# ska-telescope/ska-sdp-screen-fitting

Measured on AMD Instinct MI355X. Metric: screen-slots/sec (ant×time×freq) + FITS-cube wall-clock, KL 256² screen, higher is better.
Workload: dtype f64

## Files before the change

### include/screenfit.h

```cpp
#ifndef SCREENFIT_H
#define SCREENFIT_H

#include <stddef.h>
#include <stdint.h>

#ifdef __cplusplus
extern "C" {
#endif

#define SF_OK 0
#define SF_EINVAL (-22)
#define SF_ENOMEM (-12)
#define SF_EIO (-5)
#define SF_ENODEV (-19)

#define SF_MAX_DIR 60
#define SF_MAX_FIT_DIR 128
#define SF_MAX_EVAL_DIR 128

#define SF_SCREEN_PHASE 0
#define SF_SCREEN_TEC 1
#define SF_SCREEN_AMPLITUDE 2

#define SF_EVAL_NAN_SCRUB 1u
#define SF_EVAL_FAST_SINCOS (1u << 8)
#define SF_EVAL_NT_STORES (1u << 9)
#define SF_EVAL_BIG_ENDIAN (1u << 10)

typedef struct sf_ctx sf_ctx;

typedef struct sf_fit_params {
  int screen_type;
  int niter;
  double nsigma;
  int adjust_order;
  int ref_ant;
  int ant_offset;
  const double* ref_phase;
} sf_fit_params;

const char* sf_version(void);
const char* sf_last_error(void);
int sf_create(int device, sf_ctx** out);
int sf_destroy(sf_ctx* ctx);
int sf_set_stream(sf_ctx* ctx, void* hip_stream);
int sf_synchronize(sf_ctx* ctx);
int sf_stream_create(sf_ctx* ctx, const int* reserve_cus, int n_reserve,
                     void** hip_stream);
int sf_stream_destroy(sf_ctx* ctx, void* hip_stream);
int sf_device_cus(sf_ctx* ctx, int* n_cu);
#define SF_OPT_FIT_GENERAL 1
#define SF_OPT_EVAL_KERNEL 2
#define SF_OPT_EVAL_MAX_BLOCKS 3
#define SF_OPT_FIT_PACK 4
#define SF_OPT_EVAL_KS_PAD 5
#define SF_OPT_EVAL_SLEEP 6
#define SF_OPT_EVAL_XCD_MAP 7
#define SF_OPT_EVAL_GROUPS 8
#define SF_OPT_EVAL_BANDS 9
#define SF_OPT_FIT_LEAN 10
#define SF_OPT_TESS_SLOTS 11
#define SF_OPT_TESS_WAVES 12
#define SF_OPT_TESS_TILE 13
#define SF_OPT_TESS_BOX 14
#define SF_OPT_EVAL_INT 15
#define SF_OPT_EVAL_WG_WAVES 16
#define SF_OPT_FIT_EIG_WAVES 17
#define SF_OPT_FIT_SUBSET_DELETION 18
#define SF_OPT_FIT_WIDE_CACHE 19
#define SF_OPT_FIT_WIDE_POOL_MB 20
#define SF_OPT_FIT_WIDE_POOL_MAX 21
#define SF_OPT_FIT_LANE 22
#define SF_EVAL_KERNEL_AUTO 0
#define SF_EVAL_KERNEL_TILE 1
#define SF_EVAL_KERNEL_LDS4 2
#define SF_EVAL_KERNEL_LDS8 3
#define SF_EVAL_KERNEL_LDS16 4
#define SF_EVAL_KERNEL_LDS8H 5
#define SF_EVAL_KERNEL_LDS16H 6
#define SF_EVAL_KERNEL_TILE3 7
#define SF_EVAL_KERNEL_SHB 8
#define SF_EVAL_KERNEL_WIDE 9
int sf_get_eval_kernel(sf_ctx* ctx, int gain, unsigned flags, int* kernel);
#define SF_EVAL_CONTRACTION_F64 0
#define SF_EVAL_CONTRACTION_I8_DIGITS 1
int sf_get_eval_contraction(sf_ctx* ctx, int gain, unsigned flags, int* contraction);
int sf_set_option(sf_ctx* ctx, int option, int value);
int sf_alloc(sf_ctx* ctx, size_t bytes, void** dev_ptr);
int sf_free(sf_ctx* ctx, void* dev_ptr);
int sf_copy_h2d(sf_ctx* ctx, void* dst_dev, const void* src_host, size_t bytes);
int sf_copy_d2h(sf_ctx* ctx, void* dst_host, const void* src_dev, size_t bytes);

int sf_set_basis(sf_ctx* ctx, const double* pp_host, int D, double r0,
                 double beta);
int sf_set_basis_wide(sf_ctx* ctx, const double* pp_host, int D, double r0,
                      double beta);
int sf_get_basis(sf_ctx* ctx, double* c_host, double* pinv_c_host,
                 double* u_host, double* eig_host);

int sf_set_piercepoints(sf_ctx* ctx, const double* pp_host, int D, double r0,
                        double beta);

int sf_kl_fit(sf_ctx* ctx, const double* phase, const float* weight, int T,
              int F, int A, const int* station_order_host,
              const sf_fit_params* params, double* coef, double* resid,
              float* w_out, int32_t* order_out);

int sf_get_fit_stats(sf_ctx* ctx, int* n_masks, int* n_general);

int sf_get_fit_lane_stats(sf_ctx* ctx, int64_t* n_lane, int64_t* n_deferred);

int sf_get_fit_pool(sf_ctx* ctx, uint64_t* masks_host, double* entries_host,
                    int max_masks, int* n_masks);
int sf_get_fit_pool_wide(sf_ctx* ctx, uint64_t* masks_host, double* entries_host,
                         int max_masks, int* n_masks);

int sf_set_grid(sf_ctx* ctx, const double* x_host, int nx,
                const double* y_host, int ny);

int sf_kl_eval(sf_ctx* ctx, const double* coef, int64_t S, float* out,
               int64_t ring_slots, unsigned flags);

int sf_kl_eval_gain(sf_ctx* ctx, const double* coef_phase,
                    const double* coef_xx, const double* coef_yy, int64_t S,
                    float* out, int64_t ring_slots, unsigned flags);
int sf_kl_eval_sums(sf_ctx* ctx, const double* coef_phase,
                    const double* coef_xx, const double* coef_yy, int64_t S,
                    float* out, int64_t ring, unsigned flags,
                    uint32_t* slot_sums);

int sf_kl_eval_values(sf_ctx* ctx, const double* coef, int64_t S, float* out,
                      int64_t ring_slots, unsigned flags);

int sf_kl_eval_pol(sf_ctx* ctx, const double* phase_xx, const double* phase_yy,
                   const double* amp_xx, const double* amp_yy, int64_t S,
                   float* out, int64_t ring_slots, unsigned flags);

#define SF_MAX_TEC_FREQ 4096
int sf_set_tec_freqs(sf_ctx* ctx, const double* rad_per_tecu_host,
                     const int* tec_index_host, int F, int F_tec);
int sf_kl_eval_tec(sf_ctx* ctx, const double* tec_coef, const double* phase_coef,
                   int64_t T, int A, float* out, unsigned flags);

#define SF_MAX_POINTS 4096
int sf_set_points(sf_ctx* ctx, const double* xy_host, int P);
int sf_kl_eval_points(sf_ctx* ctx, const double* coef_phase, const double* coef_xx,
                      const double* coef_yy, int64_t S, float* planes, unsigned flags);
int sf_kl_eval_point_values(sf_ctx* ctx, const double* coef, int64_t S, double* values);

int sf_tess_fill(sf_ctx* ctx, const int32_t* labels, int nx, int ny,
                 const double* phase, const double* amp_xx,
                 const double* amp_yy, int D, int64_t S, float* out,
                 int64_t ring_slots, double smooth_pix, unsigned flags);
int sf_tess_fill_pol(sf_ctx* ctx, const int32_t* labels, int nx, int ny,
                     const double* phase, const double* phase_yy,
                     const double* amp_xx, const double* amp_yy, int D, int64_t S,
                     float* out, int64_t ring_slots, double smooth_pix,
                     unsigned flags);

int sf_smooth(sf_ctx* ctx, float* cube, int nx, int ny, int64_t n_img,
              double smooth_pix, unsigned flags);

#ifdef __cplusplus
}
#endif
#endif
```

### ska-sdp-screen-fitting_amd/csrc/capi.hip

```cpp
#include <hip/hip_runtime.h>

#include <algorithm>
#include <cmath>
#include <cstring>
#include <string>
#include <vector>

#include "sf_internal.h"

namespace sf {
static thread_local std::string g_last_error;
void set_error(const std::string& msg) { g_last_error = msg; }
}

using sf::set_error;

namespace {

int check_device(int device) {
  int n = 0;
  hipError_t e = hipGetDeviceCount(&n);
  if (e != hipSuccess || n == 0) {
    set_error("no HIP device available");
    return SF_ENODEV;
  }
  if (device < 0 || device >= n) {
    set_error("device index out of range");
    return SF_EINVAL;
  }
  hipDeviceProp_t prop;
  SF_HIP(hipGetDeviceProperties(&prop, device));
  if (std::strncmp(prop.gcnArchName, "gfx950", 6) != 0) {
    set_error(std::string("libscreenfit is built for gfx950, found ") +
              prop.gcnArchName);
    return SF_ENODEV;
  }
  return SF_OK;
}

template <typename T>
int rebind(sf::DevBuf<T>& b, size_t count) {
  b.reset();
  return b.reserve(count, "hipMalloc failed");
}

void drop_wide(sf_ctx* ctx) {
  ctx->wide = 0;
  ctx->d_wide_ws.reset();
  ctx->d_wkeys.reset();
  ctx->d_wslot.reset();
  ctx->d_wtab.reset();
  ctx->d_wtab_id.reset();
  ctx->d_wpool_mask.reset();
  ctx->d_wpool.reset();
  ctx->wide_pool_n = 0;
}

void drop_geometry(sf_ctx* ctx) {
  ctx->D = 0;
  ctx->has_basis = 0;
  drop_wide(ctx);
  ctx->nx = ctx->ny = 0;
  ctx->n_pix = 0;
  ctx->n_points = 0;
}

}

extern "C" {

const char* sf_version(void) { return "screenfit 0.1.0 (gfx950)"; }

const char* sf_last_error(void) { return sf::g_last_error.c_str(); }

int sf_create(int device, sf_ctx** out) {
  SF_REQUIRE(out != nullptr, SF_EINVAL, "sf_create: out is NULL");
  SF_TRY(check_device(device));
  SF_HIP(hipSetDevice(device));
  sf_ctx* ctx = new sf_ctx();
  ctx->device = device;
  if (ctx->d_trash.reserve(256, "sf_create: hipMalloc failed") != SF_OK) {
    delete ctx;
    return SF_ENOMEM;
  }
  *out = ctx;
  return SF_OK;
}

int sf_destroy(sf_ctx* ctx) {
  if (!ctx) return SF_OK;
  hipSetDevice(ctx->device);
  if (ctx->kdig_read) (void)hipEventDestroy(ctx->kdig_read);
  delete ctx;
  return SF_OK;
}

int sf_set_stream(sf_ctx* ctx, void* stream) {
  SF_REQUIRE(ctx, SF_EINVAL, "sf_set_stream: NULL context");
  ctx->stream = reinterpret_cast<hipStream_t>(stream);
  return SF_OK;
}

int sf_device_cus(sf_ctx* ctx, int* n_cu) {
  SF_REQUIRE(ctx && n_cu, SF_EINVAL, "sf_device_cus: NULL argument");
  SF_HIP(hipDeviceGetAttribute(n_cu, hipDeviceAttributeMultiprocessorCount,
                               ctx->device));
  return SF_OK;
}

int sf_stream_create(sf_ctx* ctx, const int* reserve_cus, int n_reserve,
                     void** stream) {
  SF_REQUIRE(ctx && stream && n_reserve >= 0 && (n_reserve == 0 || reserve_cus),
             SF_EINVAL, "sf_stream_create: bad argument");
  SF_HIP(hipSetDevice(ctx->device));
  int n_cu = 0;
  SF_TRY(sf_device_cus(ctx, &n_cu));
  hipStream_t s = nullptr;
  if (n_reserve == 0) {
    SF_HIP(hipStreamCreateWithFlags(&s, hipStreamNonBlocking));
  } else {
    std::vector<uint32_t> mask((n_cu + 31) / 32, 0u);
    for (int c = 0; c < n_cu; ++c) mask[c >> 5] |= 1u << (c & 31);
    for (int k = 0; k < n_reserve; ++k) {
      const int c = reserve_cus[k];
      SF_REQUIRE(c >= 0 && c < n_cu, SF_EINVAL, "sf_stream_create: CU index out of range");
      mask[c >> 5] &= ~(1u << (c & 31));
    }
    SF_REQUIRE(n_reserve < n_cu, SF_EINVAL, "sf_stream_create: no CU left");
    SF_HIP(hipExtStreamCreateWithCUMask(&s, (uint32_t)mask.size(), mask.data()));
  }
  *stream = s;
  return SF_OK;
}

int sf_stream_destroy(sf_ctx* ctx, void* stream) {
  SF_REQUIRE(ctx && stream, SF_EINVAL, "sf_stream_destroy: bad argument");
  SF_HIP(hipSetDevice(ctx->device));
  SF_HIP(hipStreamDestroy(reinterpret_cast<hipStream_t>(stream)));
  return SF_OK;
}

int sf_set_option(sf_ctx* ctx, int option, int value) {
  SF_REQUIRE(ctx, SF_EINVAL, "sf_set_option: NULL context");
  switch (option) {
    case SF_OPT_FIT_GENERAL:
      ctx->force_general = value != 0;
      return SF_OK;
    case SF_OPT_EVAL_KERNEL:
      SF_REQUIRE(value >= SF_EVAL_KERNEL_AUTO && value <= SF_EVAL_KERNEL_WIDE,
                 SF_EINVAL, "sf_set_option: unknown evaluation kernel");
      ctx->eval_kernel = value;
      return SF_OK;
    case SF_OPT_FIT_PACK:
      ctx->fit_pack = value != 0;
      return SF_OK;
    case SF_OPT_FIT_LEAN:
      ctx->fit_lean = value != 0;
      return SF_OK;
    case SF_OPT_FIT_LANE:
      ctx->fit_lane = value != 0;
      return SF_OK;
    case SF_OPT_EVAL_KS_PAD:
      SF_REQUIRE(value >= 0 && value <= 3, SF_EINVAL,
                 "sf_set_option: k-step padding must be 0..3");
      ctx->eval_ks_pad = value;
      return SF_OK;
    case SF_OPT_EVAL_SLEEP:
      SF_REQUIRE(value >= 0 && value <= 1000, SF_EINVAL,
                 "sf_set_option: eval sleep must be 0..1000");
      ctx->eval_sleep = value;
      return SF_OK;
    case SF_OPT_EVAL_XCD_MAP:
      SF_REQUIRE(value >= -1 && value <= 1, SF_EINVAL,
                 "sf_set_option: XCD map must be -1, 0 or 1");
      ctx->eval_xcd_map = value;
      return SF_OK;
    case SF_OPT_EVAL_GROUPS:
      SF_REQUIRE(value >= 0 && value <= 256 && (value & (value - 1)) == 0,
                 SF_EINVAL, "sf_set_option: groups must be 0 or a power of two <= 256");
      ctx->eval_groups = value;
      return SF_OK;
    case SF_OPT_EVAL_BANDS:
      SF_REQUIRE(value >= 0 && value <= 128 && (value & (value - 1)) == 0,
                 SF_EINVAL, "sf_set_option: bands must be 0 or a power of two <= 128");
      ctx->eval_bands = value;
      return SF_OK;
    case SF_OPT_TESS_SLOTS:
      SF_REQUIRE(value >= 0 && value <= 256, SF_EINVAL,
                 "sf_set_option: tess slots must be 0..256");
      ctx->tess_slots = value;
      return SF_OK;
    case SF_OPT_TESS_TILE:
      SF_REQUIRE(value == 0 || value == 1, SF_EINVAL, "sf_set_option: tess tile must be 0 or 1");
      ctx->tess_tile = value;
      return SF_OK;
    case SF_OPT_TESS_BOX:
      SF_REQUIRE(value >= -1 && value <= 1, SF_EINVAL,
                 "sf_set_option: tess box must be -1, 0 or 1");
      ctx->tess_box = value;
      return SF_OK;
    case SF_OPT_TESS_WAVES:
      SF_REQUIRE(value == 0 || value == 4 || value == 8 || value == 16, SF_EINVAL,
                 "sf_set_option: tess waves must be 0, 4, 8 or 16");
      ctx->tess_waves = value;
      return SF_OK;
    case SF_OPT_EVAL_MAX_BLOCKS:
      SF_REQUIRE(value >= 0, SF_EINVAL, "sf_set_option: negative block cap");
      ctx->eval_max_blocks = value;
      return SF_OK;
    case SF_OPT_EVAL_INT:
      SF_REQUIRE(value == -1 || value == 0, SF_EINVAL,
                 "sf_set_option: eval int must be -1 or 0");
      ctx->eval_int = value;
      return SF_OK;
    case SF_OPT_EVAL_WG_WAVES:
      SF_REQUIRE(value == 0 || value == 4 || value == 8, SF_EINVAL,
                 "sf_set_option: eval workgroup waves must be 0, 4 or 8");
      ctx->eval_wg_waves = value;
      return SF_OK;
    case SF_OPT_FIT_SUBSET_DELETION:
      SF_REQUIRE(value >= 0 && value <= 3, SF_EINVAL,
                 "SF_OPT_FIT_SUBSET_DELETION must be 0, 1, 2 or 3");
      ctx->fit_subset_deletion = (int)value;
      return SF_OK;
    case SF_OPT_FIT_EIG_WAVES:
      SF_REQUIRE(value >= 0 && value <= 4, SF_EINVAL,
                 "sf_set_option: fit eig waves must be 0..4");
      ctx->fit_eig_waves = value;
      return SF_OK;
    case SF_OPT_FIT_WIDE_CACHE:
      SF_REQUIRE(value == 0 || value == 1, SF_EINVAL,
                 "sf_set_option: fit wide cache must be 0 or 1");
      ctx->wide_cache = value;
      return SF_OK;
    case SF_OPT_FIT_WIDE_POOL_MB:
      SF_REQUIRE(value >= 0 && value <= 65536, SF_EINVAL,
                 "sf_set_option: fit wide pool MiB must be 0..65536");
      ctx->wide_pool_mb = value;
      return SF_OK;
    case SF_OPT_FIT_WIDE_POOL_MAX:
      SF_REQUIRE(value >= 0, SF_EINVAL,
                 "sf_set_option: negative fit wide pool entry cap");
      ctx->wide_pool_max = value;
      return SF_OK;
    default:
      set_error("sf_set_option: unknown option");
      return SF_EINVAL;
  }
}

int sf_get_eval_kernel(sf_ctx* ctx, int gain, unsigned flags, int* kernel) {
  SF_REQUIRE(ctx && kernel, SF_EINVAL, "sf_get_eval_kernel: bad argument");
  SF_REQUIRE(ctx->ksteps > 0, SF_EINVAL,
             "sf_get_eval_kernel: call sf_set_grid first");
  *kernel = sf::pick_eval_kernel(ctx, gain != 0, flags, true);
  return SF_OK;
}

int sf_get_eval_contraction(sf_ctx* ctx, int gain, unsigned flags, int* contraction) {
  SF_REQUIRE(ctx && contraction, SF_EINVAL, "sf_get_eval_contraction: bad argument");
  SF_REQUIRE(ctx->ksteps > 0, SF_EINVAL,
             "sf_get_eval_contraction: call sf_set_grid first");
  *contraction = sf::eval_int_applies(ctx, gain != 0, flags, true)
                     ? SF_EVAL_CONTRACTION_I8_DIGITS
                     : SF_EVAL_CONTRACTION_F64;
  return SF_OK;
}

int sf_synchronize(sf_ctx* ctx) {
  SF_REQUIRE(ctx, SF_EINVAL, "sf_synchronize: NULL context");
  SF_HIP(hipSetDevice(ctx->device));
  SF_HIP(hipStreamSynchronize(ctx->stream));
  return SF_OK;
}

int sf_alloc(sf_ctx* ctx, size_t bytes, void** p) {
  SF_REQUIRE(ctx && p, SF_EINVAL, "sf_alloc: bad argument");
  SF_HIP(hipSetDevice(ctx->device));
  if (hipMalloc(p, bytes) != hipSuccess) {
    set_error("sf_alloc: hipMalloc failed");
    return SF_ENOMEM;
  }
  return SF_OK;
}

int sf_free(sf_ctx* ctx, void* p) {
  SF_REQUIRE(ctx, SF_EINVAL, "sf_free: NULL context");
  SF_HIP(hipSetDevice(ctx->device));
  SF_HIP(hipFree(p));
  return SF_OK;
}

int sf_copy_h2d(sf_ctx* ctx, void* dst, const void* src, size_t bytes) {
  SF_REQUIRE(ctx && (bytes == 0 || (dst && src)), SF_EINVAL,
             "sf_copy_h2d: bad argument");
  SF_HIP(hipSetDevice(ctx->device));
  SF_HIP(hipMemcpyAsync(dst, src, bytes, hipMemcpyHostToDevice, ctx->stream));
  SF_HIP(hipStreamSynchronize(ctx->stream));
  return SF_OK;
}

int sf_copy_d2h(sf_ctx* ctx, void* dst, const void* src, size_t bytes) {
  SF_REQUIRE(ctx && (bytes == 0 || (dst && src)), SF_EINVAL,
             "sf_copy_d2h: bad argument");
  SF_HIP(hipSetDevice(ctx->device));
  SF_HIP(hipMemcpyAsync(dst, src, bytes, hipMemcpyDeviceToHost, ctx->stream));
  SF_HIP(hipStreamSynchronize(ctx->stream));
  return SF_OK;
}

int sf_set_basis(sf_ctx* ctx, const double* pp, int D, double r0,
                 double beta) {
  SF_REQUIRE(ctx && pp, SF_EINVAL, "sf_set_basis: bad argument");
  SF_REQUIRE(D >= 1 && D <= SF_MAX_DIR, SF_EINVAL,
             "sf_set_basis: D out of range [1, SF_MAX_DIR]");
  SF_REQUIRE(r0 > 0.0, SF_EINVAL, "sf_set_basis: r0 must be > 0");
  SF_HIP(hipSetDevice(ctx->device));
  SF_HIP(hipStreamSynchronize(ctx->stream));
  drop_geometry(ctx);
  SF_TRY(rebind(ctx->d_pp, (size_t)3 * D));
  SF_TRY(rebind(ctx->d_c, (size_t)D * D));
  SF_TRY(rebind(ctx->d_pinv, (size_t)D * D));
  SF_TRY(rebind(ctx->d_u, (size_t)D * D));
  SF_TRY(rebind(ctx->d_eig, (size_t)64));
  SF_HIP(hipMemcpy(ctx->d_pp, pp, sizeof(double) * 3 * D,
                   hipMemcpyHostToDevice));
  for (int i = 0; i < 3 * D; ++i) ctx->h_pp[i] = pp[i];
  SF_HIP(hipMemset(ctx->d_eig, 0, 64 * sizeof(double)));
  ctx->D = D;
  ctx->r0 = r0;
  ctx->beta = beta;
  int rc = sf::launch_basis(ctx);
  if (rc == SF_OK && hipStreamSynchronize(ctx->stream) != hipSuccess) {
    set_error("sf_set_basis: basis kernel failed");
    rc = SF_EIO;
  }
  if (rc != SF_OK) ctx->D = 0;
  ctx->has_basis = rc == SF_OK;
  return rc;
}

int sf_set_piercepoints(sf_ctx* ctx, const double* pp, int D, double r0,
                        double beta) {
  SF_REQUIRE(ctx && pp, SF_EINVAL, "sf_set_piercepoints: bad argument");
  SF_REQUIRE(D >= 1 && D <= SF_MAX_EVAL_DIR, SF_EINVAL,
             "sf_set_piercepoints: D out of range [1, SF_MAX_EVAL_DIR]");
  SF_REQUIRE(r0 > 0.0, SF_EINVAL, "sf_set_piercepoints: r0 must be > 0");
  SF_HIP(hipSetDevice(ctx->device));
  SF_HIP(hipStreamSynchronize(ctx->stream));
  drop_geometry(ctx);
  SF_TRY(rebind(ctx->d_pp, (size_t)3 * D));
  SF_HIP(hipMemcpy(ctx->d_pp, pp, sizeof(double) * 3 * D,
                   hipMemcpyHostToDevice));
  for (int i = 0; i < 3 * D; ++i) ctx->h_pp[i] = pp[i];
  ctx->D = D;
  ctx->r0 = r0;
  ctx->beta = beta;
  return SF_OK;
}

int sf_set_basis_wide(sf_ctx* ctx, const double* pp, int D, double r0,
                      double beta) {
  SF_REQUIRE(ctx && pp, SF_EINVAL, "sf_set_basis_wide: bad argument");
  SF_REQUIRE(D >= 1 && D <= SF_MAX_FIT_DIR, SF_EINVAL,
             "sf_set_basis_wide: D out of range [1, SF_MAX_FIT_DIR]");
  if (D <= SF_MAX_DIR) return sf_set_basis(ctx, pp, D, r0, beta);
  SF_TRY(sf_set_piercepoints(ctx, pp, D, r0, beta));
  drop_geometry(ctx);
  SF_TRY(rebind(ctx->d_c, (size_t)D * D));
  SF_TRY(rebind(ctx->d_pinv, (size_t)D * D));
  SF_TRY(rebind(ctx->d_u, (size_t)D * D));
  SF_TRY(rebind(ctx->d_eig, (size_t)SF_MAX_FIT_DIR));
  SF_HIP(hipMemset(ctx->d_eig, 0, SF_MAX_FIT_DIR * sizeof(double)));
  ctx->D = D;
  int rc = sf::launch_basis_wide(ctx);
  if (rc == SF_OK && hipStreamSynchronize(ctx->stream) != hipSuccess) {
    set_error("sf_set_basis_wide: basis kernel failed");
    rc = SF_EIO;
  }
  if (rc != SF_OK) ctx->D = 0;
  ctx->has_basis = rc == SF_OK;
  ctx->wide = rc == SF_OK;
  return rc;
}

int sf_get_basis(sf_ctx* ctx, double* c, double* pinv, double* u,
                 double* eig) {
  SF_REQUIRE(ctx && ctx->D > 0, SF_EINVAL, "sf_get_basis: no basis set");
  SF_REQUIRE(ctx->has_basis, SF_EINVAL,
             "sf_get_basis: the context holds piercepoints only "
             "(sf_set_piercepoints); call sf_set_basis");
  SF_HIP(hipSetDevice(ctx->device));
  SF_HIP(hipStreamSynchronize(ctx->stream));
  const size_t n = (size_t)ctx->D * ctx->D * sizeof(double);
  if (c) SF_HIP(hipMemcpy(c, ctx->d_c, n, hipMemcpyDeviceToHost));
  if (pinv) SF_HIP(hipMemcpy(pinv, ctx->d_pinv, n, hipMemcpyDeviceToHost));
  if (u) SF_HIP(hipMemcpy(u, ctx->d_u, n, hipMemcpyDeviceToHost));
  if (eig)
    SF_HIP(hipMemcpy(eig, ctx->d_eig, ctx->D * sizeof(double),
                     hipMemcpyDeviceToHost));
  return SF_OK;
}

int sf_kl_fit(sf_ctx* ctx, const double* phase, const float* weight, int T,
              int F, int A, const int* st_order, const sf_fit_params* p,
              double* coef, double* resid, float* w_out, int32_t* order_out) {
  SF_REQUIRE(ctx && ctx->D > 0, SF_EINVAL, "sf_kl_fit: call sf_set_basis first");
  SF_REQUIRE(ctx->has_basis, SF_EINVAL,
             "sf_kl_fit: the context holds piercepoints only "
             "(sf_set_piercepoints); the fit needs sf_set_basis");
  SF_REQUIRE(phase && weight && st_order && p && coef, SF_EINVAL,
             "sf_kl_fit: NULL argument");
  SF_REQUIRE(T >= 1 && F >= 1 && A >= 1, SF_EINVAL,
             "sf_kl_fit: T, F, A must be >= 1");
  SF_REQUIRE((int64_t)F * A <= INT32_MAX / 2, SF_EINVAL,
             "sf_kl_fit: F * A too large");
  SF_REQUIRE(p->screen_type == SF_SCREEN_PHASE || p->screen_type == SF_SCREEN_TEC ||
                 p->screen_type == SF_SCREEN_AMPLITUDE,
             SF_EINVAL, "sf_kl_fit: unsupported screen type");
  SF_REQUIRE(p->niter >= 1 && p->niter <= 64, SF_EINVAL,
             "sf_kl_fit: niter must be in [1, 64]");
  SF_REQUIRE((int64_t)T * F * A * (2 * p->niter + 2) < ((int64_t)1 << 30),
             SF_EINVAL,
             "sf_kl_fit: too many slots for one call (split the time axis)");
  SF_REQUIRE(p->ref_ant >= -1 && p->ant_offset >= 0, SF_EINVAL,
             "sf_kl_fit: bad ref_ant / ant_offset");
  {
    const int rl = p->ref_ant - p->ant_offset;
    SF_REQUIRE(p->ref_ant == -1 || p->ref_phase || (rl >= 0 && rl < A),
               SF_EINVAL,
               "sf_kl_fit: reference station not in this shard and no "
               "ref_phase given");
  }
  for (int a = 0; a < A; ++a)
    SF_REQUIRE(st_order[a] >= 0, SF_EINVAL, "sf_kl_fit: negative order");
  SF_HIP(hipSetDevice(ctx->device));
  SF_TRY(ctx->d_skip.reserve((size_t)F * A, "hipMalloc failed"));
  SF_TRY(ctx->d_st_order.reserve((size_t)A, "hipMalloc failed"));
  SF_HIP(hipMemcpyAsync(ctx->d_st_order, st_order, sizeof(int) * A,
                        hipMemcpyHostToDevice, ctx->stream));
  return sf::launch_fit(ctx, phase, weight, T, F, A, p, coef, resid, w_out,
                        order_out);
}

int sf_get_fit_stats(sf_ctx* ctx, int* n_masks, int* n_general) {
  SF_REQUIRE(ctx, SF_EINVAL, "sf_get_fit_stats: NULL context");
  int c[sf::kFitCounters] = {};
  SF_HIP(hipSetDevice(ctx->device));
  SF_HIP(hipStreamSynchronize(ctx->stream));
  if (ctx->d_counters)
    SF_HIP(hipMemcpy(c, ctx->d_counters, sizeof(c), hipMemcpyDeviceToHost));
  static_assert(sf::kCntIds == sf::kCntWideDecomp, "n_masks reads one slot");
  if (n_masks) *n_masks = c[sf::kCntIds];
  if (n_general) *n_general = c[sf::kCntSlow];
  return SF_OK;
}

int sf_get_fit_lane_stats(sf_ctx* ctx, int64_t* n_lane, int64_t* n_deferred) {
  SF_REQUIRE(ctx, SF_EINVAL, "sf_get_fit_lane_stats: NULL context");
  int c[sf::kFitCounters] = {};
  SF_HIP(hipSetDevice(ctx->device));
  SF_HIP(hipStreamSynchronize(ctx->stream));
  if (ctx->d_counters)
    SF_HIP(hipMemcpy(c, ctx->d_counters, sizeof(c), hipMemcpyDeviceToHost));
  if (n_lane) *n_lane = c[sf::kCntLane];
  if (n_deferred) *n_deferred = c[sf::kCntLaneDeferred];
  return SF_OK;
}

int sf_get_fit_pool(sf_ctx* ctx, uint64_t* masks_host, double* entries_host,
                    int max_masks, int* n_masks) {
  SF_REQUIRE(ctx && n_masks && max_masks >= 0, SF_EINVAL, "sf_get_fit_pool: bad argument");
  SF_REQUIRE(max_masks == 0 || (masks_host && entries_host), SF_EINVAL,
             "sf_get_fit_pool: NULL output");
  SF_REQUIRE(!ctx->wide, SF_EINVAL,
             "sf_get_fit_pool: 64-bit mask keys; above SF_MAX_DIR directions "
             "(sf_set_basis_wide) call sf_get_fit_pool_wide");
  SF_HIP(hipSetDevice(ctx->device));
  SF_HIP(hipStreamSynchronize(ctx->stream));
  int c0 = 0;
  if (ctx->d_counters)
    SF_HIP(hipMemcpy(&c0, ctx->d_counters + sf::kCntIds, sizeof(int),
                     hipMemcpyDeviceToHost));
  const int n = ctx->pool_D == ctx->D && (size_t)c0 <= ctx->d_pool_mask.size() ? c0 : 0;
  *n_masks = n;
  const int k = n < max_masks ? n : max_masks;
  if (k > 0) {
    const size_t entry = (size_t)ctx->D * ctx->D + ctx->D;
    SF_HIP(hipMemcpy(masks_host, ctx->d_pool_mask, k * sizeof(uint64_t),
                     hipMemcpyDeviceToHost));
    SF_HIP(hipMemcpy(entries_host, ctx->d_pool, k * entry * sizeof(double),
                     hipMemcpyDeviceToHost));
  }
  return SF_OK;
}

int sf_get_fit_pool_wide(sf_ctx* ctx, uint64_t* masks_host, double* entries_host,
                         int max_masks, int* n_masks) {
  SF_REQUIRE(ctx && n_masks && max_masks >= 0, SF_EINVAL,
             "sf_get_fit_pool_wide: bad argument");
  SF_REQUIRE(max_masks == 0 || (masks_host && entries_host), SF_EINVAL,
             "sf_get_fit_pool_wide: NULL output");
  SF_REQUIRE(ctx->wide && ctx->has_basis, SF_EINVAL,
             "sf_get_fit_pool_wide: the context holds no wide basis "
             "(sf_set_basis_wide with more than SF_MAX_DIR directions)");
  SF_HIP(hipSetDevice(ctx->device));
  SF_HIP(hipStreamSynchronize(ctx->stream));
  const int n = ctx->wide_pool_n;
  *n_masks = n;
  const int k = n < max_masks ? n : max_masks;
  if (k > 0) return sf::read_fit_pool_wide(ctx, masks_host, entries_host, k);
  return SF_OK;
}

int sf_set_grid(sf_ctx* ctx, const double* x, int nx, const double* y,
                int ny) {
  SF_REQUIRE(ctx && ctx->D > 0, SF_EINVAL,
             "sf_set_grid: call sf_set_basis or sf_set_piercepoints first");
  SF_REQUIRE(x && y && nx >= 1 && ny >= 1, SF_EINVAL, "sf_set_grid: bad grid");
  for (int i = 0; i < nx; ++i)
    SF_REQUIRE(std::isfinite(x[i]), SF_EINVAL, "sf_set_grid: non-finite x coordinate");
  for (int j = 0; j < ny; ++j)
    SF_REQUIRE(std::isfinite(y[j]), SF_EINVAL, "sf_set_grid: non-finite y coordinate");
  SF_REQUIRE((int64_t)nx * ny <= ((int64_t)1 << 31), SF_EINVAL,
             "sf_set_grid: grid too large");
  SF_HIP(hipSetDevice(ctx->device));
  ctx->n_pix = 0;
  ctx->nx = nx;
  ctx->ny = ny;
  const int64_t n_pix = (int64_t)nx * ny;
  ctx->n_pix_blocks = (n_pix + sf::kBlockPix - 1) / sf::kBlockPix;
  ctx->ksteps = (ctx->D + 3) / 4;
  const size_t n = (size_t)ctx->n_pix_blocks * sf::kEvalWaves * ctx->ksteps *
                   sf::kTiles * 64;
  SF_TRY(rebind(ctx->d_cfrag, n));
  sf::DevBuf<double> dx, dy;
  sf::DevBuf<int> dbad;
  SF_TRY(dx.reserve((size_t)nx, "hipMalloc failed"));
  SF_TRY(dy.reserve((size_t)ny, "hipMalloc failed"));
  int rc = SF_OK;
  if (hipMemcpyAsync(dx, x, sizeof(double) * nx, hipMemcpyHostToDevice,
                     ctx->stream) != hipSuccess ||
      hipMemcpyAsync(dy, y, sizeof(double) * ny, hipMemcpyHostToDevice,
                     ctx->stream) != hipSuccess) {
    set_error("sf_set_grid: copy of the grid coordinates failed");
    rc = SF_EIO;
  } else {
    rc = sf::launch_cpix(ctx, dx, dy);
  }
  double cmax = 0.0;
  for (int d = 0; d < ctx->D; ++d) {
    const double px = ctx->h_pp[3 * d], py = ctx->h_pp[3 * d + 1];
    double mx = 0.0, my = 0.0, nxd = HUGE_VAL, nyd = HUGE_VAL;
    for (int i = 0; i < nx; ++i) {
      mx = std::fmax(mx, std::fabs(px - x[i]));
      nxd = std::fmin(nxd, std::fabs(px - x[i]));
    }
    for (int j = 0; j < ny; ++j) {
      my = std::fmax(my, std::fabs(py - y[j]));
      nyd = std::fmin(nyd, std::fabs(py - y[j]));
    }
    const double z = ctx->h_pp[3 * d + 2];
    for (const double d2 : {mx * mx + my * my + z * z, nxd * nxd + nyd * nyd + z * z}) {
      const double c = 1.01 * 0.5 * std::pow(d2 / (ctx->r0 * ctx->r0), ctx->beta / 2.0);
      cmax = std::isfinite(c) ? std::fmax(cmax, c) : HUGE_VAL;
    }
  }
  ctx->dig_ok = 0;
  if (rc == SF_OK && ctx->ksteps >= 12 && ctx->ksteps <= sf::kEvalMaxKS &&
      std::isfinite(cmax) &&
      cmax * 68719476736.0 < std::ldexp(1.0, 46) * 1.86) {
    if (rebind(ctx->d_cdig, (size_t)ctx->n_pix_blocks * sf::kEvalWaves * sf::kDigits *
                                sf::kTiles * 64 * 16) == SF_OK &&
        dbad.reserve(1, "hipMalloc failed") == SF_OK &&
        hipMemsetAsync(dbad, 0, sizeof(int), ctx->stream) == hipSuccess) {
      rc = sf::launch_cdig(ctx, dx, dy, dbad);
      if (rc == SF_OK) ctx->dig_ok = 1;
    }
  }
  if (hipStreamSynchronize(ctx->stream) != hipSuccess && rc == SF_OK) {
    set_error("sf_set_grid: pixel basis kernel failed");
    rc = SF_EIO;
  }
  if (ctx->dig_ok) {
    int bad = 1;
    if (hipMemcpy(&bad, dbad, sizeof(int), hipMemcpyDeviceToHost) != hipSuccess || bad)
      ctx->dig_ok = 0;
  }
  if (rc == SF_OK) {
    ctx->rev_thr = cmax > 0.0 && std::isfinite(cmax) ? 32768.0 / cmax : 0.0;
    ctx->n_pix = n_pix;
  } else {
    ctx->dig_ok = 0;
  }
  return rc;
}

int sf_kl_eval(sf_ctx* ctx, const double* coef, int64_t S, float* out,
               int64_t ring, unsigned flags) {
  SF_REQUIRE(ctx && ctx->n_pix > 0 && ctx->d_cfrag, SF_EINVAL,
             "sf_kl_eval: call sf_set_grid first");
  SF_REQUIRE(coef && out && S >= 0 && ring >= 1, SF_EINVAL,
             "sf_kl_eval: bad argument");
  if (S == 0) return SF_OK;
  SF_HIP(hipSetDevice(ctx->device));
  return sf::launch_eval(ctx, coef, nullptr, nullptr, S, out, ring, flags,
                         nullptr);
}

int sf_kl_eval_gain(sf_ctx* ctx, const double* coef_phase,
                    const double* coef_xx, const double* coef_yy, int64_t S,
                    float* out, int64_t ring, unsigned flags) {
  SF_REQUIRE(ctx && ctx->n_pix > 0 && ctx->d_cfrag, SF_EINVAL,
             "sf_kl_eval_gain: call sf_set_grid first");
  SF_REQUIRE(coef_phase && coef_xx && coef_yy && out && S >= 0 && ring >= 1,
             SF_EINVAL, "sf_kl_eval_gain: bad argument");
  if (S == 0) return SF_OK;
  SF_HIP(hipSetDevice(ctx->device));
  return sf::launch_eval(ctx, coef_phase, coef_xx, coef_yy, S, out, ring, flags,
                         nullptr);
}

int sf_kl_eval_sums(sf_ctx* ctx, const double* coef_phase,
                    const double* coef_xx, const double* coef_yy, int64_t S,
                    float* out, int64_t ring, unsigned flags,
                    uint32_t* slot_sums) {
  SF_REQUIRE(ctx && ctx->n_pix > 0 && ctx->d_cfrag, SF_EINVAL,
             "sf_kl_eval_sums: call sf_set_grid first");
  SF_REQUIRE(coef_phase && out && slot_sums && S >= 0 && ring >= 1,
             SF_EINVAL, "sf_kl_eval_sums: bad argument");
  SF_REQUIRE((coef_xx == nullptr) == (coef_yy == nullptr), SF_EINVAL,
             "sf_kl_eval_sums: give both amplitude coefficient sets or neither");
  if (S == 0) return SF_OK;
  SF_HIP(hipSetDevice(ctx->device));
  return sf::launch_eval(ctx, coef_phase, coef_xx, coef_yy, S, out, ring, flags,
                         reinterpret_cast<unsigned*>(slot_sums));
}

int sf_set_points(sf_ctx* ctx, const double* xy, int P) {
  SF_REQUIRE(ctx, SF_EINVAL, "sf_set_points: NULL context");
  SF_REQUIRE(ctx->D > 0, SF_EINVAL,
             "sf_set_points: call sf_set_basis, sf_set_basis_wide or "
             "sf_set_piercepoints first");
  SF_REQUIRE(xy, SF_EINVAL, "sf_set_points: NULL positions");
  SF_REQUIRE(P >= 1 && P <= SF_MAX_POINTS, SF_EINVAL,
             "sf_set_points: P out of range [1, SF_MAX_POINTS]");
  for (int i = 0; i < 2 * P; ++i)
    SF_REQUIRE(std::isfinite(xy[i]), SF_EINVAL, "sf_set_points: non-finite coordinate");
  SF_HIP(hipSetDevice(ctx->device));
  SF_HIP(hipStreamSynchronize(ctx->stream));
  ctx->n_points = 0;
  if (ctx->pt_cus == 0) SF_TRY(sf_device_cus(ctx, &ctx->pt_cus));
  const int tiles = sf::points_tiles(P), ks_pad = sf::points_ks_pad(ctx->D);
  SF_TRY(rebind(ctx->d_pxy, (size_t)2 * P));
  SF_TRY(rebind(ctx->d_pfrag, (size_t)tiles * ks_pad * 64));
  SF_HIP(hipMemcpy(ctx->d_pxy, xy, sizeof(double) * 2 * P, hipMemcpyHostToDevice));
  ctx->pt_tiles = tiles;
  ctx->pt_ks_pad = ks_pad;
  ctx->n_points = P;
  int rc = sf::launch_points_cpix(ctx);
  if (rc == SF_OK && hipStreamSynchronize(ctx->stream) != hipSuccess) {
    set_error("sf_set_points: point basis kernel failed");
    rc = SF_EIO;
  }
  if (rc != SF_OK) ctx->n_points = 0;
  return rc;
}

int sf_kl_eval_points(sf_ctx* ctx, const double* coef_phase, const double* coef_xx,
                      const double* coef_yy, int64_t S, float* planes,
                      unsigned flags) {
  SF_REQUIRE(ctx, SF_EINVAL, "sf_kl_eval_points: NULL context");
  SF_REQUIRE(ctx->D > 0 && ctx->n_points > 0 && ctx->d_pfrag, SF_EINVAL,
             "sf_kl_eval_points: call sf_set_points first");
  SF_REQUIRE(coef_phase && planes, SF_EINVAL, "sf_kl_eval_points: NULL argument");
  SF_REQUIRE((coef_xx == nullptr) == (coef_yy == nullptr), SF_EINVAL,
             "sf_kl_eval_points: give both amplitude coefficient sets or neither");
  SF_REQUIRE(S >= 1, SF_EINVAL, "sf_kl_eval_points: S must be >= 1");
  SF_REQUIRE((flags & ~(SF_EVAL_NAN_SCRUB | SF_EVAL_FAST_SINCOS)) == 0, SF_EINVAL,
             "sf_kl_eval_points: flags other than SF_EVAL_NAN_SCRUB and "
             "SF_EVAL_FAST_SINCOS");
  SF_HIP(hipSetDevice(ctx->device));
  return sf::launch_eval_points(ctx, coef_phase, coef_xx, coef_yy, S, planes, flags);
}

int sf_kl_eval_point_values(sf_ctx* ctx, const double* coef, int64_t S,
                            double* values) {
  SF_REQUIRE(ctx, SF_EINVAL, "sf_kl_eval_point_values: NULL context");
  SF_REQUIRE(ctx->D > 0 && ctx->n_points > 0 && ctx->d_pfrag, SF_EINVAL,
             "sf_kl_eval_point_values: call sf_set_points first");
  SF_REQUIRE(coef && values, SF_EINVAL, "sf_kl_eval_point_values: NULL argument");
  SF_REQUIRE(S >= 1, SF_EINVAL, "sf_kl_eval_point_values: S must be >= 1");
  SF_HIP(hipSetDevice(ctx->device));
  return sf::launch_eval_point_values(ctx, coef, S, values);
}

int sf_kl_eval_values(sf_ctx* ctx, const double* coef, int64_t S, float* out,
                      int64_t ring, unsigned flags) {
  SF_REQUIRE(ctx, SF_EINVAL, "sf_kl_eval_values: NULL context");
  SF_REQUIRE(ctx->D > 0 && ctx->n_pix > 0 && ctx->d_cfrag, SF_EINVAL,
             "sf_kl_eval_values: call sf_set_grid first");
  SF_REQUIRE(coef && out && S >= 0 && ring >= 1, SF_EINVAL,
             "sf_kl_eval_values: bad argument");
  SF_REQUIRE((reinterpret_cast<uintptr_t>(out) & 3) == 0, SF_EINVAL,
             "sf_kl_eval_values: output not 4-byte aligned");
  SF_REQUIRE((flags & ~(SF_EVAL_NAN_SCRUB | SF_EVAL_NT_STORES | SF_EVAL_BIG_ENDIAN)) == 0,
             SF_EINVAL,
             "sf_kl_eval_values: flags other than SF_EVAL_NAN_SCRUB, "
             "SF_EVAL_NT_STORES and SF_EVAL_BIG_ENDIAN");
  if (S == 0) return SF_OK;
  SF_HIP(hipSetDevice(ctx->device));
  return sf::launch_eval_values(ctx, coef, S, out, ring, flags);
}

int sf_kl_eval_pol(sf_ctx* ctx, const double* phase_xx, const double* phase_yy,
                   const double* amp_xx, const double* amp_yy, int64_t S, float* out,
                   int64_t ring, unsigned flags) {
  SF_REQUIRE(ctx, SF_EINVAL, "sf_kl_eval_pol: NULL context");
  SF_REQUIRE(ctx->D > 0 && ctx->n_pix > 0 && ctx->d_cfrag, SF_EINVAL,
             "sf_kl_eval_pol: call sf_set_grid first");
  SF_REQUIRE(phase_xx && phase_yy, SF_EINVAL,
             "sf_kl_eval_pol: both phase coefficient sets are required");
  SF_REQUIRE((amp_xx == nullptr) == (amp_yy == nullptr), SF_EINVAL,
             "sf_kl_eval_pol: give both amplitude coefficient sets or neither");
  SF_REQUIRE(out && S >= 0 && ring >= 1, SF_EINVAL, "sf_kl_eval_pol: bad argument");
  SF_REQUIRE((reinterpret_cast<uintptr_t>(out) & 3) == 0, SF_EINVAL,
             "sf_kl_eval_pol: output not 4-byte aligned");
  SF_REQUIRE((flags & ~(SF_EVAL_NAN_SCRUB | SF_EVAL_FAST_SINCOS | SF_EVAL_NT_STORES |
                        SF_EVAL_BIG_ENDIAN)) == 0,
             SF_EINVAL,
             "sf_kl_eval_pol: flags other than SF_EVAL_NAN_SCRUB, SF_EVAL_FAST_SINCOS, "
             "SF_EVAL_NT_STORES and SF_EVAL_BIG_ENDIAN");
  if (S == 0) return SF_OK;
  SF_HIP(hipSetDevice(ctx->device));
  return sf::launch_eval_pol(ctx, phase_xx, phase_yy, amp_xx, amp_yy, S, out, ring, flags);
}

int sf_set_tec_freqs(sf_ctx* ctx, const double* rad_per_tecu, const int* tec_index,
                     int F, int F_tec) {
  SF_REQUIRE(ctx, SF_EINVAL, "sf_set_tec_freqs: NULL context");
  SF_REQUIRE(rad_per_tecu, SF_EINVAL, "sf_set_tec_freqs: NULL scales");
  SF_REQUIRE(F >= 1 && F <= SF_MAX_TEC_FREQ, SF_EINVAL,
             "sf_set_tec_freqs: F out of range [1, SF_MAX_TEC_FREQ]");
  SF_REQUIRE(F_tec >= 1, SF_EINVAL, "sf_set_tec_freqs: F_tec must be >= 1");
  for (int f = 0; f < F; ++f) {
    SF_REQUIRE(std::isfinite(rad_per_tecu[f]), SF_EINVAL,
               "sf_set_tec_freqs: non-finite scale");
    SF_REQUIRE(!tec_index || (tec_index[f] >= 0 && tec_index[f] < F_tec), SF_EINVAL,
               "sf_set_tec_freqs: TEC frequency index out of range [0, F_tec)");
  }
  std::vector<double> k(F);
  std::vector<int> ch(F), order(F);
  for (int f = 0; f < F; ++f) order[f] = f;
  std::stable_sort(order.begin(), order.end(), [&](int a, int b) {
    return (tec_index ? tec_index[a] : 0) < (tec_index ? tec_index[b] : 0);
  });
  std::vector<int> used, off(1, 0);
  for (int c = 0; c < F; ++c) {
    const int f = order[c], i = tec_index ? tec_index[f] : 0;
    if (used.empty() || used.back() != i) {
      if (!used.empty()) off.push_back(c);
      used.push_back(i);
    }
    k[c] = rad_per_tecu[f] / 6.283185307179586;
    ch[c] = f;
  }
  off.push_back(F);
  SF_HIP(hipSetDevice(ctx->device));
  SF_HIP(hipStreamSynchronize(ctx->stream));
  sf::DevBuf<double> d;
  SF_TRY(d.reserve((size_t)F + (F + 1) / 2, "sf_set_tec_freqs: hipMalloc failed"));
  if (hipMemcpy(d, k.data(), F * sizeof(double), hipMemcpyHostToDevice) != hipSuccess ||
      hipMemcpy(d + F, ch.data(), F * sizeof(int), hipMemcpyHostToDevice) != hipSuccess) {
    set_error("sf_set_tec_freqs: copy of the channel lists failed");
    return SF_EIO;
  }
  ctx->d_tec_ch.swap(d);
  ctx->tec_F = F;
  ctx->tec_F_tec = F_tec;
  ctx->tec_used.swap(used);
  ctx->tec_off.swap(off);
  return SF_OK;
}

int sf_kl_eval_tec(sf_ctx* ctx, const double* tec_coef, const double* phase_coef,
                   int64_t T, int A, float* out, unsigned flags) {
  SF_REQUIRE(ctx, SF_EINVAL, "sf_kl_eval_tec: NULL context");
  SF_REQUIRE(ctx->D > 0 && ctx->n_pix > 0 && ctx->d_cfrag, SF_EINVAL,
             "sf_kl_eval_tec: call sf_set_grid first");
  SF_REQUIRE(ctx->tec_F > 0 && ctx->d_tec_ch, SF_EINVAL,
             "sf_kl_eval_tec: call sf_set_tec_freqs first");
  SF_REQUIRE(tec_coef && out && T >= 0 && A >= 1, SF_EINVAL,
             "sf_kl_eval_tec: bad argument");
  SF_REQUIRE(T * A <= INT32_MAX, SF_EINVAL,
             "sf_kl_eval_tec: T * A too large for one call (split the time axis)");
  SF_REQUIRE((reinterpret_cast<uintptr_t>(out) & 3) == 0, SF_EINVAL,
             "sf_kl_eval_tec: output not 4-byte aligned");
  SF_REQUIRE((flags & ~(SF_EVAL_NAN_SCRUB | SF_EVAL_FAST_SINCOS | SF_EVAL_NT_STORES |
                        SF_EVAL_BIG_ENDIAN)) == 0,
             SF_EINVAL,
             "sf_kl_eval_tec: flags other than SF_EVAL_NAN_SCRUB, SF_EVAL_FAST_SINCOS, "
             "SF_EVAL_NT_STORES and SF_EVAL_BIG_ENDIAN");
  if (T == 0) return SF_OK;
  SF_HIP(hipSetDevice(ctx->device));
  return sf::launch_eval_tec(ctx, tec_coef, phase_coef, T, A, out, flags);
}

static int upload_gaussian(sf_ctx* ctx, double sigma, int* R_out) {
  if (sigma <= 1e-15) sigma = 0.0;
  const int R = sigma > 0.0 ? (int)(4.0 * sigma + 0.5) : 0;
  *R_out = R;
  if (ctx->d_gw && sigma == ctx->gw_sigma) return SF_OK;
  std::vector<double> w(1, 1.0);
  if (sigma > 0.0) {
    w.assign(2 * R + 1, 0.0);
    double sum = 0.0;
    for (int i = -R; i <= R; ++i)
      w[i + R] = std::exp(-0.5 / (sigma * sigma) * (double)(i * i));
    for (int i = 0; i < 2 * R + 1; ++i) sum += w[i];
    for (int i = 0; i < 2 * R + 1; ++i) w[i] /= sum;
  }
  SF_HIP(hipDeviceSynchronize());
  ctx->gw_sigma = -1.0;
  SF_TRY(ctx->d_gw.reserve(w.size() < 64 ? 64 : w.size(), "hipMalloc failed"));
  SF_HIP(hipMemcpyAsync(ctx->d_gw, w.data(), w.size() * sizeof(double),
                        hipMemcpyHostToDevice, ctx->stream));
  SF_HIP(hipStreamSynchronize(ctx->stream));
  ctx->gw_sigma = sigma;
  return SF_OK;
}

int sf_tess_fill(sf_ctx* ctx, const int32_t* labels, int nx, int ny,
                 const double* phase, const double* amp_xx,
                 const double* amp_yy, int D, int64_t S, float* out,
                 int64_t ring, double smooth_pix, unsigned flags) {
  return sf_tess_fill_pol(ctx, labels, nx, ny, phase, nullptr, amp_xx, amp_yy, D, S, out, ring,
                          smooth_pix, flags);
}

int sf_tess_fill_pol(sf_ctx* ctx, const int32_t* labels, int nx, int ny,
                     const double* phase, const double* phase_yy, const double* amp_xx,
                     const double* amp_yy, int D, int64_t S, float* out,
                     int64_t ring, double smooth_pix, unsigned flags) {
  SF_REQUIRE(ctx && labels && phase && out, SF_EINVAL, "sf_tess_fill: NULL argument");
  SF_REQUIRE(nx >= 1 && ny >= 1 && D >= 1 && D <= SF_MAX_EVAL_DIR && S >= 0 && ring >= 1 &&
                 ring <= INT32_MAX,
             SF_EINVAL, "sf_tess_fill: bad shape");
  SF_REQUIRE(smooth_pix >= 0.0 && smooth_pix <= 1e4, SF_EINVAL,
             "sf_tess_fill: smooth_pix must be in [0, 1e4]");
  if (S == 0) return SF_OK;
  SF_HIP(hipSetDevice(ctx->device));
  int R = 0;
  int rc = upload_gaussian(ctx, smooth_pix, &R);
  if (rc != SF_OK) return rc;
  if (R <= sf::kTessMaxR)
    return (ctx->tess_tile ? sf::launch_tess_tile : sf::launch_tess)(
        ctx, labels, nx, ny, phase, phase_yy, amp_xx, amp_yy, D, S, out, ring, ctx->d_gw, R,
        flags);
  SF_REQUIRE(ring >= S, SF_EINVAL,
             "sf_tess_fill: smooth_pix > 6 needs ring_slots >= S");
  rc = sf::launch_tess(ctx, labels, nx, ny, phase, phase_yy, amp_xx, amp_yy, D, S, out,
                       ring, ctx->d_gw, 0, 0u);
  if (rc != SF_OK) return rc;
  return sf::launch_smooth(ctx, out, nx, ny, S * 4, ctx->d_gw, R, flags);
}

int sf_smooth(sf_ctx* ctx, float* cube, int nx, int ny, int64_t n_img,
              double smooth_pix, unsigned flags) {
  SF_REQUIRE(ctx && cube && nx >= 1 && ny >= 1 && n_img >= 0, SF_EINVAL,
             "sf_smooth: bad argument");
  SF_REQUIRE(n_img % 4 == 0, SF_EINVAL,
             "sf_smooth: n_img must count whole [4][ny][nx] slot cubes");
  SF_REQUIRE(smooth_pix >= 0.0 && smooth_pix <= 1e4, SF_EINVAL,
             "sf_smooth: smooth_pix must be in [0, 1e4]");
  if (n_img == 0) return SF_OK;
  SF_HIP(hipSetDevice(ctx->device));
  int R = 0;
  const int rc = upload_gaussian(ctx, smooth_pix, &R);
  if (rc != SF_OK) return rc;
  return sf::launch_smooth(ctx, cube, nx, ny, n_img, ctx->d_gw, R, flags);
}

}
```

### ska-sdp-screen-fitting_amd/csrc/kl_fit_fast.hip

```cpp
#include <hip/hip_runtime.h>

#include <cmath>
#include <cstdlib>

#include "kl_fit_lane.h"
#include "kl_fit_pool.h"
#include "kl_fit_steps.h"
#include "sf_internal.h"

namespace sf {

constexpr size_t kLdsBytes = 160 * 1024;
constexpr double kTinyW = kPinvAtol * 1.001;

template <int GW>
__global__ __launch_bounds__(256) void kl_classify_kernel(
    const float* __restrict__ weight, int64_t S, int F, int A, int D,
    const int* __restrict__ st_order, const uint8_t* __restrict__ skip,
    int ref_skip, unsigned long long* __restrict__ keys, int cap,
    int* __restrict__ pos, uint8_t* __restrict__ cls,
    int* __restrict__ counters,
    double* __restrict__ coef, double* __restrict__ resid,
    float* __restrict__ w_out, int32_t* __restrict__ order_out, int lane_fit) {
  constexpr int kPerWave = 64 / GW;
  const int l = lane();
  const int g = l / GW;
  const int d = l % GW;
  const int64_t s = ((int64_t)blockIdx.x * (blockDim.x / 64) + threadIdx.x / 64) *
                        kPerWave + g;
  const bool live = s < S && d < D;
  float x = 0.0f;
  if (live) {
    x = weight[s * D + d];
    w_out[s * D + d] = x;
  }
  const unsigned long long bm = __ballot(live && x > 0.0f);
  const unsigned long long bt = __ballot(live && x > 0.0f && (double)x <= kTinyW);
  const unsigned long long gmask = (GW == 64) ? ~0ull : ((1ull << GW) - 1ull);
  const unsigned long long mask = (bm >> (g * GW)) & gmask;
  const bool tiny = ((bt >> (g * GW)) & gmask) != 0ull;
  const float w_first = __shfl(x, g * GW + (mask ? __builtin_ctzll(mask) : 0));
  const unsigned long long bn = __ballot(live && x > 0.0f && x != w_first);
  const bool nonuniform = ((bn >> (g * GW)) & gmask) != 0ull;
  if (s >= S) return;
  const SlotGeom sg(s, F, A);
  const bool skipped = sg.skipped(skip, ref_skip);
  if (live && skipped) {
    coef[s * D + d] = 0.0;
    resid[s * D + d] = 0.0;
  }
  if (d != 0) return;
  if (skipped) {
    cls[s] = kClassSkipped;
    order_out[s] = 0;
    pos[s] = -2;
    return;
  }
  order_out[s] = st_order[sg.a];
  if (tiny) atomicAdd(counters + kCntSlow, 1);
  else if (nonuniform) atomicAdd(counters + kCntNonUniform, 1);
  const bool to_lane = lane_fit && !tiny && !nonuniform && mask == full_mask(D);
  cls[s] = tiny ? kClassSlow : to_lane ? kClassLane : kClassFast;
  if (mask == full_mask(D)) pos[s] = -1;
  else if (mask == 0ull) pos[s] = -2;
  else pos[s] = table_insert(keys, cap, mask);
}

struct FastLds {
  const double* U;
  const double* C;
  int cld;
  const double* lam;
  double* Vs;
  double* lams;
  double* G;
  double* M;
  double* vec;
  double2* cs;
  int2* pr;
  __device__ void jacobi(double* a, double* v, int n, int ld) const {
    wave_jacobi(a, v, cs, pr, n, ld, kJacobiMaxSweeps);
  }
};

__host__ __device__ inline size_t fast_shared_bytes(int D, bool c_global) {
  return (size_t)((c_global ? 1 : 2) * D * odd_ld(D) + 64) * sizeof(double);
}
__host__ __device__ inline size_t fast_wave_bytes(int D, bool slow, bool lean = false) {
  if (lean) return (size_t)6 * 64 * sizeof(double);
  return (size_t)((slow ? 3 : 2) * D * odd_ld(D) + 64 + 6 * 64) * sizeof(double) +
         (slow ? 64 * sizeof(double2) + 96 * sizeof(int2) : 0);
}

struct Basis {
  int n;
  bool full;
  int ld;
  const double* U;
  const double* lam;
};

template <bool SLOW, int SPW, bool LEAN>
__device__ void fit_once(const FastLds& L, const Basis& B, int D, int ld,
                         int K, int screen_type, bool uniform, double wu,
                         double phi_p, double w_p, double phi_d, double w_d,
                         double& white_d, double& resid_d) {
#pragma clang fp contract(off)
  using G = Group<SPW>;
  using M = FitMath<!SLOW>;
  constexpr int kMatVecUnroll = LEAN ? 4 : 1;
  const int l = G::lane();
  const int n = B.n;
  double* v0 = L.vec;
  double* v1 = L.vec + 64;
  double* v2 = L.vec + 128;
  double* v3 = L.vec + 192;
  double rc = 0.0, rs = 0.0;
  if (l < n) {
    if (screen_type == SF_SCREEN_PHASE) {
      double sn, cn;
      M::sin_cos(phi_p, &sn, &cn);
      rc = w_p * cn;
      rs = w_p * sn;
    } else if (screen_type == SF_SCREEN_AMPLITUDE) {
      rc = w_p * M::lg10(phi_p);
    } else {
      rc = w_p * phi_p;
    }
    v0[l] = rc;
    v1[l] = rs;
    v2[l] = w_p;
  }
  lds_sync();
  const Tie2 tie(n, K, v0, v1, v2, B.lam);
  double a1 = 0.0, a2 = 0.0;
  if (l < K) {
#pragma unroll kMatVecUnroll
    for (int p = 0; p < n; ++p) {
      const double u = B.U[p * B.ld + l];
      a1 += u * v0[p];
      a2 += u * v1[p];
    }
  }
  if (K > 0) {
    if (!SLOW && (LEAN || uniform)) {
      a1 /= wu;
      a2 /= wu;
    } else {
      if (l < K) {
        for (int j = 0; j < K; ++j) {
          double s = 0.0;
          for (int p = 0; p < n; ++p)
            s += B.U[p * B.ld + l] * (v2[p] * B.U[p * B.ld + j]);
          L.G[l * ld + j] = s;
        }
      }
      lds_sync();
      if (!SLOW) {
        wave_cholesky_solve2<SPW>(L.G, K, ld, a1, a2);
      } else {
        truncated_eig_solve(G{}, L, L.G, L.M, K, ld, v0, v1, v2, v3, a1, a2);
      }
    }
  }
  lds_sync();
  if (l < K) {
    const bool keep = fabs(B.lam[l]) > kPinvAtol;
    v0[l] = keep ? a1 : 0.0;
    v1[l] = keep ? a2 : 0.0;
  }
  lds_sync();
  double screen = 0.0;
  if (l < n) {
    double cre = 0.0, cim = 0.0;
#pragma unroll kMatVecUnroll
    for (int k = 0; k < K; ++k) {
      const double u = B.U[l * B.ld + k];
      cre += u * v0[k];
      cim += u * v1[k];
    }
    screen = (screen_type == SF_SCREEN_PHASE) ? M::arctan2(cim, cre) : cre;
    if (tie.on) screen = tie.template screen<M>(screen_type, l);
  }
  lds_sync();
  if (l < n) v2[l] = screen;
  lds_sync();
  if (l < n) {
    double sh = 0.0;
#pragma unroll kMatVecUnroll
    for (int p = 0; p < n; ++p) sh += B.U[p * B.ld + l] * v2[p];
    const double lm = B.lam[l];
    const bool keep = fabs(lm) > kPinvAtol;
    v0[l] = keep ? sh / lm : 0.0;
    v1[l] = keep ? sh : 0.0;
  }
  lds_sync();
  double white = 0.0, cw = 0.0;
  if (l < n) {
#pragma unroll kMatVecUnroll
    for (int r = 0; r < n; ++r) {
      const double u = B.U[l * B.ld + r];
      white += u * v0[r];
      cw += u * v1[r];
    }
  }
  lds_sync();
  if (B.full) {
    white_d = white;
    resid_d = phi_d - model_value<M>(screen_type, cw);
    return;
  }
  if (l < n) {
    v0[l] = screen;
    v1[l] = white;
  }
  lds_sync();
  const bool unfl = (l < D) && (w_d > 0.0);
  const unsigned long long m = G::ballot(unfl);
  double sall = 0.0;
  if (l < D) {
    if (unfl) {
      const int p = G::rank(m);
      sall = v0[p];
    } else {
      unsigned long long mm = m;
      int p = 0;
      while (mm) {
        const int q = __builtin_ctzll(mm);
        sall += L.C[l * L.cld + q] * v1[p];
        mm &= mm - 1;
        ++p;
      }
    }
  }
  lds_sync();
  if (l < D) v2[l] = sall;
  lds_sync();
  if (l < D) {
    double sh = 0.0;
#pragma unroll kMatVecUnroll
    for (int p = 0; p < D; ++p) sh += L.U[p * ld + l] * v2[p];
    const double lm = L.lam[l];
    v0[l] = fabs(lm) > kPinvAtol ? sh / lm : 0.0;
  }
  lds_sync();
  double wa = 0.0;
  if (l < D)
#pragma unroll kMatVecUnroll
    for (int r = 0; r < D; ++r) wa += L.U[l * ld + r] * v0[r];
  lds_sync();
  white_d = wa;
  resid_d = phi_d - model_value<M>(screen_type, sall);
}

#ifndef SF_FIT_MINW
#define SF_FIT_MINW 4
#endif
template <bool SLOW, int SPW, bool LEAN>
__global__ __launch_bounds__(256, SLOW ? 1 : SF_FIT_MINW) void kl_fit_pass_kernel(
    int it, int niter, int64_t S, int F, int A, int D,
    const double* __restrict__ phase, const double* __restrict__ refph,
    int ref_sub, const double* __restrict__ g_u, const double* __restrict__ g_c,
    const double* __restrict__ g_eig, const int* __restrict__ st_order,
    const uint8_t* __restrict__ cls, int* __restrict__ pos,
    const int* __restrict__ ids, unsigned long long* __restrict__ keys, int cap,
    const double* __restrict__ pool, int pool_cap, int* __restrict__ counters,
    int screen_type, double nsigma, int adjust_order, double* __restrict__ coef,
    double* __restrict__ resid, float* __restrict__ w_out,
    int32_t* __restrict__ order_out, const long long* __restrict__ list) {
#pragma clang fp contract(off)
  extern __shared__ double smem[];
  const int ld = odd_ld(D);
  using G = Group<SPW>;
  using M = FitMath<!SLOW>;
  const G tm;
  constexpr bool CG = SPW == 1;
  const int nwaves = blockDim.x / 64;
  const int nslots = nwaves * SPW;
  const int wv = (threadIdx.x / 64) * SPW + G::index();
  const int d = G::lane();
  double* sU = smem;
  double* sC = CG ? nullptr : sU + D * ld;
  double* sl = sU + (CG ? 1 : 2) * D * ld;
  for (int e = threadIdx.x; e < D * D; e += blockDim.x) {
    const int r = e / D, c = e % D;
    sU[r * ld + c] = g_u[e];
    if (!CG) sC[r * ld + c] = g_c[e];
  }
  for (int e = threadIdx.x; e < 64; e += blockDim.x) sl[e] = e < D ? g_eig[e] : 0.0;
  __syncthreads();
  FastLds L;
  L.U = sU;
  L.C = CG ? g_c : sC;
  L.cld = CG ? D : ld;
  L.lam = sl;
  double* wb = sl + 64 + (size_t)wv * (fast_wave_bytes(D, SLOW, LEAN) / sizeof(double));
  if (LEAN) {
    L.Vs = L.G = L.M = L.lams = nullptr;
    L.vec = wb;
    L.cs = nullptr;
    L.pr = nullptr;
  } else {
    L.Vs = wb;
    L.G = wb + D * ld;
    L.M = L.G + D * ld;
    L.lams = (SLOW ? L.M + D * ld : L.G + D * ld);
    L.vec = L.lams + 64;
    L.cs = reinterpret_cast<double2*>(L.vec + 6 * 64);
    L.pr = reinterpret_cast<int2*>(L.cs + 64);
  }
  const uint8_t want = SLOW ? 2 : 0;

  const int64_t n_work = list ? (int64_t)counters[kCntList] : S;
  for (int64_t i = (int64_t)blockIdx.x * nslots + wv; i < n_work;
       i += (int64_t)gridDim.x * nslots) {
    int64_t s = i;
    if (list) {
      const long long e = list[i];
      if (list_first(e) > it) continue;
      s = list_slot(e);
    }
    if (SLOW && cls[s] != want) continue;
    const uint8_t cl = SLOW ? want : cls[s];
    const int a = (int)(s % A);
    const int p0 = pos[s];
    const int64_t base = s * D;
    double phi_d = 0.0, w_d = 0.0, white_d = 0.0, resid_d = 0.0;
    if (d < D) {
      phi_d = phase_ref(phase, refph, ref_sub, s, a, A, D, d);
      w_d = (double)w_out[base + d];
      white_d = it == 0 ? 0.0 : coef[base + d];
      resid_d = it == 0 ? 0.0 : resid[base + d];
    }
    double order = (double)order_out[s];
    const double station_order = (double)st_order[a];
    if (cl != want) continue;
    int id = -1;
    if (p0 >= 0) {
      id = ids[p0];
      if (id < 0 || id >= pool_cap) {
        if (d == 0) atomicOr(counters + kCntError, kErrLookupMiss);
        continue;
      }
    } else if (p0 == -3) {
      if (d == 0) atomicOr(counters + kCntError, kErrTableFull);
      continue;
    }
    const bool unfl = (d < D) && (w_d > 0.0);
    const unsigned long long um = G::ballot(unfl);
    const int n_unfl = __popcll(um);

    Basis B;
    B.n = n_unfl;
    B.full = (n_unfl == D);
    B.ld = ld;
    if (B.full) {
      B.U = L.U;
      B.lam = L.lam;
    } else if (n_unfl > 0) {
      const double* e = pool + (size_t)id * (D * D + D);
      if (LEAN) {
        B.U = e;
        B.ld = D;
        B.lam = e + D * D;
      } else {
        for (int r = 0; r < n_unfl; ++r)
          if (d < n_unfl) L.Vs[r * ld + d] = e[r * D + d];
        if (d < n_unfl) L.lams[d] = e[D * D + d];
        lds_sync();
        B.U = L.Vs;
        B.lam = L.lams;
      }
    }
    double phi_p = 0.0, w_p = 0.0;
    {
      double* v4 = L.vec + 256;
      double* v5 = L.vec + 320;
      if (unfl) {
        const int p = G::rank(um);
        v4[p] = phi_d;
        v5[p] = w_d;
      }
      lds_sync();
      if (d < n_unfl) {
        phi_p = v4[d];
        w_p = v5[d];
      }
      lds_sync();
    }
    const double wmax = G::max(unfl ? w_d : -INFINITY);
    const double wmin = -G::max(unfl ? -w_d : -INFINITY);
    const bool uniform = (wmax == wmin);
    if (LEAN && n_unfl > 0 && !uniform) {
      if (d == 0) atomicOr(counters + kCntError, kErrLeanNonUniform);
      continue;
    }

    if (n_unfl > 0) {
      if (order > n_unfl - 1) order = n_unfl - 1;
      if (it == 0) {
        fit_once<SLOW, SPW, LEAN>(L, B, D, ld, (int)order, screen_type, uniform, wmin,
                       phi_p, w_p, phi_d, w_d, white_d, resid_d);
      } else if (adjust_order) {
        OrderWalk walk;
        for (int oi = 0; oi < 4; ++oi) {
          if (oi > 0)
            fit_once<SLOW, SPW, LEAN>(L, B, D, ld, (int)order, screen_type, uniform, wmin,
                           phi_p, w_p, phi_d, w_d, white_d, resid_d);
          if (walk.done()) break;
          const double redchi2 = slot_redchi2<M>(tm, screen_type, d < D, unfl, phi_d,
                                                 w_d, resid_d, n_unfl, order);
          if (walk.template step<M>(oi, redchi2, n_unfl, station_order, order)) break;
        }
      }
    }
    if (it + 1 < niter && screen_type == SF_SCREEN_PHASE) {
      const bool live = d < D;
      if (G::any(live && w_d > 0.0) &&
          G::any(flag_circular_outliers<M>(tm, live, nsigma, resid_d, w_d))) {
        const unsigned long long nm = G::ballot(live && w_d > 0.0);
        if (d == 0) pos[s] = (nm == 0ull) ? -2 : table_insert(keys, cap, nm);
      }
    }
    if (d < D) {
      coef[base + d] = white_d;
      resid[base + d] = resid_d;
      w_out[base + d] = (float)w_d;
    }
    if (d == 0) order_out[s] = (int32_t)order;
  }
}

__global__ __launch_bounds__(256) void kl_block_sigma_kernel(
    int T, int F, int A, int D, const double* __restrict__ phase,
    const double* __restrict__ refph, int ref_sub,
    const uint8_t* __restrict__ skip, int ref_skip, int screen_type,
    const double* __restrict__ resid, const float* __restrict__ w_out,
    double* __restrict__ sigma) {
  __shared__ double red[2][256];
  const int blk = blockIdx.x;
  const int f = blk / A, a = blk % A;
  double sw = 0.0, swr = 0.0;
  if (!(skip[blk] || a == ref_skip)) {
    for (int e = threadIdx.x; e < T * D; e += blockDim.x) {
      const int t = e / D, d = e % D;
      const int64_t s = ((int64_t)t * F + f) * A + a;
      const double w = (double)w_out[s * D + d];
      if (w > 0.0) {
        const double v = phase_ref(phase, refph, ref_sub, s, a, A, D, d);
        const double sd = screen_diff(screen_type, v, resid[s * D + d]);
        swr += w * (sd * sd);
        sw += w;
      }
    }
  }
  red[0][threadIdx.x] = sw;
  red[1][threadIdx.x] = swr;
  __syncthreads();
  for (int o = 128; o > 0; o >>= 1) {
    if (threadIdx.x < o) {
      red[0][threadIdx.x] += red[0][threadIdx.x + o];
      red[1][threadIdx.x] += red[1][threadIdx.x + o];
    }
    __syncthreads();
  }
  if (threadIdx.x == 0) sigma[blk] = sqrt(red[1][0] / red[0][0]);
}

__global__ __launch_bounds__(256) void kl_block_flag_kernel(
    int64_t S, int F, int A, int D, const double* __restrict__ phase,
    const double* __restrict__ refph, int ref_sub,
    const uint8_t* __restrict__ cls, int screen_type, double nsigma,
    const double* __restrict__ sigma, const double* __restrict__ resid,
    float* __restrict__ w_out, unsigned long long* __restrict__ keys, int cap,
    int* __restrict__ pos) {
  const int64_t s = (int64_t)blockIdx.x * blockDim.x + threadIdx.x;
  if (s >= S || (cls[s] != 0 && cls[s] != 2)) return;
  const SlotGeom g(s, F, A);
  const int a = g.a;
  const double sig = sigma[g.blk];
  unsigned long long m = 0ull;
  bool changed = false;
  for (int d = 0; d < D; ++d) {
    float w = w_out[s * D + d];
    const double v = phase_ref(phase, refph, ref_sub, s, a, A, D, d);
    const double sd = screen_diff(screen_type, v, resid[s * D + d]);
    if (fabs(sd) > nsigma * sig && w != 0.0f) {
      w = 0.0f;
      w_out[s * D + d] = w;
      changed = true;
    }
    if (w > 0.0f) m |= 1ull << d;
  }
  if (changed) {
    pos[s] = (m == 0ull) ? -2 : (m == full_mask(D) ? -1 : table_insert(keys, cap, m));
  }
}

static int launch_pass(sf_ctx* ctx, bool slow, int it, const sf_fit_params* p,
                       const RefSpec& r, int64_t S, int F, int A,
                       const double* phase, double* coef, double* resid,
                       float* w_out, int32_t* order_out, bool lean,
                       const long long* list) {
  const int D = ctx->D;
  const int spw = !slow && D <= 32 && ctx->fit_pack ? 2 : 1;
  lean = !slow && lean && ctx->fit_lean;
  decltype(&kl_fit_pass_kernel<false, 1, false>) const kernels[3][2] = {
      {kl_fit_pass_kernel<false, 1, false>, kl_fit_pass_kernel<false, 2, false>},
      {kl_fit_pass_kernel<false, 1, true>, kl_fit_pass_kernel<false, 2, true>},
      {kl_fit_pass_kernel<true, 1, false>, kl_fit_pass_kernel<true, 2, false>}};
  const auto kernel = kernels[slow ? 2 : lean][spw - 1];
  const size_t shared = fast_shared_bytes(D, spw == 1);
  const size_t slot = fast_wave_bytes(D, slow, lean);
  int nw = 1, best = 0;
  for (int k = 1; k <= 4; ++k) {
    const size_t per_wg = shared + (size_t)k * spw * slot;
    if (per_wg > kLdsBytes) break;
    const int waves = k * (int)(kLdsBytes / per_wg);
    if (waves > best) {
      best = waves;
      nw = k;
    }
  }
  const size_t shm = shared + (size_t)nw * spw * slot;
  SF_TRY(allow_lds(kernel, shm));
  int64_t blocks = (S + nw * spw - 1) / (nw * spw);
  if (blocks > 16384) blocks = 16384;
  hipLaunchKernelGGL(kernel, dim3((unsigned)blocks), dim3(64 * nw), shm,
                     ctx->stream, it, p->niter, S, F, A, D, phase, r.refph, r.sub,
                     ctx->d_u, ctx->d_c, ctx->d_eig, ctx->d_st_order, ctx->d_class,
                     ctx->d_pos, ctx->d_ids, ctx->d_keys, (int)ctx->d_keys.size(),
                     ctx->d_pool, (int)ctx->d_pool_mask.size(), ctx->d_counters,
                     p->screen_type, p->nsigma, p->adjust_order, coef, resid, w_out,
                     order_out, list);
  SF_HIP(hipGetLastError());
  return SF_OK;
}

int launch_block_sigma(sf_ctx* ctx, int T, int F, int A, const double* phase,
                       const RefSpec& r, int screen_type, const double* resid,
                       const float* w_out) {
  hipLaunchKernelGGL(kl_block_sigma_kernel, dim3(F * A), dim3(256), 0,
                     ctx->stream, T, F, A, ctx->D, phase, r.refph, r.sub,
                     ctx->d_skip, r.skip, screen_type, resid, w_out,
                     ctx->d_sigma);
  SF_HIP(hipGetLastError());
  return SF_OK;
}

int fit_buffers(sf_ctx* ctx, int64_t S, int F, int A, double** resid,
                float** w_out, int32_t** order_out) {
  const size_t n = (size_t)S * ctx->D;
  if (!*resid) {
    SF_TRY(ctx->d_scratch.reserve(n, kFitAlloc));
    *resid = ctx->d_scratch;
  }
  if (!*w_out) {
    SF_TRY(ctx->d_wscratch.reserve(n, kFitAlloc));
    *w_out = ctx->d_wscratch;
  }
  if (!*order_out) {
    SF_TRY(ctx->d_oscratch.reserve((size_t)S, kFitAlloc));
    *order_out = ctx->d_oscratch;
  }
  SF_TRY(ctx->d_sigma.reserve((size_t)F * A, kFitAlloc));
  SF_TRY(ctx->d_counters.reserve((size_t)kFitCounters, kFitAlloc));
  return SF_OK;
}

int launch_fit(sf_ctx* ctx, const double* phase, const float* weight, int T,
               int F, int A, const sf_fit_params* p, double* coef,
               double* resid, float* w_out, int32_t* order_out) {
  if (ctx->wide)
    return launch_fit_wide(ctx, phase, weight, T, F, A, p, coef, resid, w_out,
                           order_out);
  const int D = ctx->D;
  const int64_t S = (int64_t)T * F * A;
  const RefSpec r = ref_spec(p, A);
  SF_TRY(launch_skip(ctx, phase, weight, T, F, A, r));

  static const char* env = std::getenv("SCREENFIT_FIT");
  if (ctx->force_general || (env && env[0] == 'g')) {
    if (p->screen_type == SF_SCREEN_AMPLITUDE ||
        (p->niter > 1 && p->screen_type != SF_SCREEN_PHASE)) {
      set_error("the general fit kernel handles phase (any niter) and tec (niter 1) only");
      return SF_EINVAL;
    }
    return launch_fit_general(ctx, phase, weight, T, F, A, p, r, coef, resid,
                              w_out, order_out);
  }
  SF_TRY(fit_buffers(ctx, S, F, A, &resid, &w_out, &order_out));
  SF_TRY(reserve_pair(ctx->d_pos, (size_t)S, ctx->d_class, (size_t)S, kFitAlloc));
  const size_t tcap = next_pow2((size_t)(2 * p->niter + 2) * (size_t)S + 64, 1);
  SF_TRY(reserve_pair(ctx->d_keys, tcap, ctx->d_ids, tcap, kFitAlloc));
  SF_TRY(ensure_pool(ctx, 1024));
  const int cap = (int)ctx->d_keys.size();
  SF_HIP(hipMemsetAsync(ctx->d_keys, 0, cap * sizeof(unsigned long long), ctx->stream));
  SF_HIP(hipMemsetAsync(ctx->d_ids, 0xff, cap * sizeof(int), ctx->stream));
  SF_HIP(hipMemsetAsync(ctx->d_counters, 0, kFitCounters * sizeof(int), ctx->stream));
  const bool lane_fit = fit_lane_applies(ctx, p);
  if (lane_fit) SF_TRY(ctx->d_list.reserve((size_t)S, kFitAlloc));
  long long* const list = lane_fit ? ctx->d_list : nullptr;

  {
    const int gw = D <= 8 ? 8 : D <= 16 ? 16 : D <= 32 ? 32 : 64;
    const int64_t per_block = 4 * (64 / gw);
    const dim3 grid((unsigned)((S + per_block - 1) / per_block));
    const auto classify = gw == 8    ? kl_classify_kernel<8>
                          : gw == 16 ? kl_classify_kernel<16>
                          : gw == 32 ? kl_classify_kernel<32>
                                     : kl_classify_kernel<64>;
    hipLaunchKernelGGL(classify, grid, dim3(256), 0, ctx->stream, weight, S, F, A, D,
                       ctx->d_st_order, ctx->d_skip, r.skip, ctx->d_keys, cap,
                       ctx->d_pos, ctx->d_class, ctx->d_counters, coef, resid, w_out,
                       order_out, lane_fit ? 1 : 0);
    SF_HIP(hipGetLastError());
  }

  const bool block_flags = p->screen_type != SF_SCREEN_PHASE;
  for (int it = 0; it < p->niter; ++it) {
    int n_slow = 0, n_nonuniform = 0;
    SF_TRY(number_and_decompose(ctx, &n_slow, &n_nonuniform));
    if (it == 0 && lane_fit)
      SF_TRY(launch_fit_lane(ctx, p, r, S, A, phase, coef, resid, w_out, order_out));
    SF_TRY(launch_pass(ctx, false, it, p, r, S, F, A, phase, coef, resid, w_out,
                          order_out, n_nonuniform == 0, list));
    if (n_slow > 0)
      SF_TRY(launch_pass(ctx, true, it, p, r, S, F, A, phase, coef, resid, w_out,
                            order_out, false, nullptr));
    if (block_flags && it + 1 < p->niter) {
      SF_TRY(launch_block_sigma(ctx, T, F, A, phase, r, p->screen_type, resid,
                                 w_out));
      hipLaunchKernelGGL(kl_block_flag_kernel, dim3((unsigned)((S + 255) / 256)),
                         dim3(256), 0, ctx->stream, S, F, A, D, phase, r.refph,
                         r.sub, ctx->d_class, p->screen_type, p->nsigma,
                         ctx->d_sigma, resid, w_out, ctx->d_keys, cap,
                         ctx->d_pos);
      SF_HIP(hipGetLastError());
    }
  }
  int err = 0;
  SF_HIP(hipMemcpyAsync(&err, ctx->d_counters + kCntError, sizeof(int),
                        hipMemcpyDeviceToHost, ctx->stream));
  SF_HIP(hipStreamSynchronize(ctx->stream));
  SF_REQUIRE((err & (kErrLookupMiss | kErrTableFull)) == 0, SF_EIO,
             "sf_kl_fit: internal mask table overflow");
  SF_REQUIRE((err & kErrLeanNonUniform) == 0, SF_EIO,
             "sf_kl_fit: lean fit pass saw non-uniform weights in a slot "
             "classified uniform (slot left unwritten)");
  SF_REQUIRE((err & kErrFullMaskInPool) == 0, SF_EIO,
             "sf_kl_fit: a mask with every direction unflagged entered the "
             "subset-basis pool (its basis is the global one; left unbuilt)");
  return SF_OK;
}

}
```

### ska-sdp-screen-fitting_amd/csrc/kl_fit_lane.h

```cpp
#pragma once

#include <cstdint>

#include "sf_internal.h"

namespace sf {

constexpr uint8_t kClassFast = 0, kClassSkipped = 1, kClassSlow = 2, kClassLane = 3;

constexpr int kLaneMinD = 3;
constexpr int kLaneMaxD = 23;

constexpr int kListPassShift = 56;
__host__ __device__ inline long long list_entry(int64_t s, int first) {
  return (long long)s | ((long long)first << kListPassShift);
}
__host__ __device__ inline int64_t list_slot(long long e) {
  return (int64_t)(e & ((1ll << kListPassShift) - 1));
}
__host__ __device__ inline int list_first(long long e) {
  return (int)(e >> kListPassShift);
}

inline bool fit_lane_applies(const sf_ctx* ctx, const sf_fit_params* p) {
  return ctx->fit_lane && ctx->fit_pack && !ctx->wide &&
         p->screen_type == SF_SCREEN_PHASE && ctx->D >= kLaneMinD &&
         ctx->D <= kLaneMaxD;
}

int launch_fit_lane(sf_ctx* ctx, const sf_fit_params* p, const RefSpec& r,
                    int64_t S, int A, const double* phase, double* coef,
                    double* resid, float* w_out, int32_t* order_out);

}
```

### ska-sdp-screen-fitting_amd/csrc/kl_fit_lane.hip

```cpp
#include <hip/hip_runtime.h>

#include <cmath>

#include "kl_fit_lane.h"
#include "kl_fit_masks.h"
#include "kl_fit_steps.h"
#include "sf_internal.h"

#pragma clang fp contract(off)

namespace sf {

using LaneMath = FitMath<false>;


template <int D, class Leaf>
__device__ __forceinline__ void tree_sum3(double (&out)[3], Leaf leaf) {
  static_assert(D <= 32, "a half-wave of directions");
  double t5[3] = {0.0, 0.0, 0.0};
#pragma unroll 1
  for (int b0 = 0; b0 < 2; ++b0) {
    double t4[3] = {0.0, 0.0, 0.0};
#pragma unroll 1
    for (int b1 = 0; b1 < 2; ++b1) {
      double t3[3] = {0.0, 0.0, 0.0};
#pragma unroll 1
      for (int b2 = 0; b2 < 2; ++b2) {
        double t2[3] = {0.0, 0.0, 0.0};
#pragma unroll 1
        for (int b3 = 0; b3 < 2; ++b3) {
          double t1[3] = {0.0, 0.0, 0.0};
#pragma unroll 1
          for (int b4 = 0; b4 < 2; ++b4) {
            const int p = b0 + 2 * b1 + 4 * b2 + 8 * b3 + 16 * b4;
            double x[3] = {0.0, 0.0, 0.0};
            if (p < D) leaf(p, x);
#pragma unroll
            for (int k = 0; k < 3; ++k) t1[k] = b4 == 0 ? x[k] : t1[k] + x[k];
          }
#pragma unroll
          for (int k = 0; k < 3; ++k) t2[k] = b3 == 0 ? t1[k] : t2[k] + t1[k];
        }
#pragma unroll
        for (int k = 0; k < 3; ++k) t3[k] = b2 == 0 ? t2[k] : t3[k] + t2[k];
      }
#pragma unroll
      for (int k = 0; k < 3; ++k) t4[k] = b1 == 0 ? t3[k] : t4[k] + t3[k];
    }
#pragma unroll
    for (int k = 0; k < 3; ++k) t5[k] = b0 == 0 ? t4[k] : t5[k] + t4[k];
  }
#pragma unroll
  for (int k = 0; k < 3; ++k) out[k] = t5[k];
}

template <int D, int LDX, class T>
__device__ __forceinline__ void store_rows(T* dst, const double* X, int n_elem,
                                           unsigned long long rows) {
  for (int e = lane(); e < n_elem; e += 64) {
    const int r = e / D, d = e % D;
    if ((rows >> r) & 1ull) dst[e] = (T)X[d * LDX + r];
  }
}

constexpr int kGroups = 16;
__global__ __launch_bounds__(256) void kl_lane_list_kernel(
    const uint8_t* __restrict__ cls, int64_t S, int* __restrict__ counters,
    long long* __restrict__ list) {
  const int l = lane();
  const int64_t sb = ((int64_t)blockIdx.x * (blockDim.x / 64) + threadIdx.x / 64) *
                     (64 * kGroups);
  if (sb >= S) return;
  int my_at[kGroups];
  int n_fast = 0, n_lane = 0;
#pragma unroll
  for (int g = 0; g < kGroups; ++g) {
    const int64_t sg = sb + g * 64 + l;
    const uint8_t c = sg < S ? cls[sg] : kClassSkipped;
    const unsigned long long fast_rows = __ballot(c == kClassFast);
    my_at[g] = c == kClassFast ? n_fast + Group<1>::rank(fast_rows) : -1;
    n_fast += __popcll(fast_rows);
    n_lane += __popcll(__ballot(c == kClassLane));
  }
  unsigned long long old = 0ull;
  if (l == 0 && (n_fast | n_lane) != 0)
    old = atomicAdd(reinterpret_cast<unsigned long long*>(counters + kCntLane),
                    (unsigned long long)n_lane | ((unsigned long long)n_fast << 32));
  const int base = (int)(__shfl(old, 0) >> 32);
#pragma unroll
  for (int g = 0; g < kGroups; ++g)
    if (my_at[g] >= 0) list[base + my_at[g]] = list_entry(sb + g * 64 + l, 0);
}

template <int D>
__global__ __launch_bounds__(64, 2) void kl_fit_lane_kernel(
    int niter, int64_t S, int A, const double* __restrict__ phase,
    const double* __restrict__ refph, int ref_sub,
    const double* __restrict__ g_u, const double* __restrict__ g_eig,
    const int* __restrict__ st_order, uint8_t* __restrict__ cls,
    int* __restrict__ pos, unsigned long long* __restrict__ keys, int cap,
    int* __restrict__ counters, long long* __restrict__ list, double nsigma,
    int adjust_order, double* __restrict__ coef, double* __restrict__ resid,
    float* __restrict__ w_out, int32_t* __restrict__ order_out) {
  constexpr int LDX = 65;
  __shared__ double X[D * LDX];
  __shared__ double sU[D * D + D];
  __shared__ long long row_tf[64];
  __shared__ int row_a[64];
  const int l = lane();
  const int64_t s0 = (int64_t)blockIdx.x * 64;
  const int64_t s = s0 + l;
  const bool mine = s < S && cls[s] == kClassLane;
  if (__ballot(mine) == 0ull) return;
  const int n_elem = (int)(S - s0 < 64 ? S - s0 : 64) * D;
  const int a = (int)(s % A);
  const double* sLam = sU + D * D;
  for (int e = l; e < D * D; e += 64) sU[e] = g_u[e];
  if (l < D) sU[D * D + l] = g_eig[l];
  row_a[l] = a;
  row_tf[l] = (long long)(s / A);
  lds_sync();
  for (int e = l; e < n_elem; e += 64) {
    const int r = e / D, d = e % D;
    double v = phase[s0 * D + e];
    if (refph) v -= refph[row_tf[r] * D + d];
    else if (ref_sub >= 0) v -= phase[(s0 + r + (ref_sub - row_a[r])) * D + d];
    X[d * LDX + r] = v;
  }
  lds_sync();
  double* x = X + l;

  bool run = mine;
  int defer = -1;
  if (run) {
    bool finite = true;
#pragma unroll 1
    for (int p = 0; p < D; ++p) finite = finite && __builtin_isfinite(x[p * LDX]);
    if (!finite) {
      defer = 0;
      run = false;
    }
  }
  const bool fitted = run;
  const double wu = mine ? (double)w_out[s * D] : 1.0;
  const double station_order = mine ? (double)st_order[a] : 0.0;
  double order = station_order;

  if (run) {
    if (order > D - 1) order = D - 1;
    const int K = (int)order;
    double v0[D], v1[D];
#pragma unroll
    for (int k = 0; k < D; ++k) v0[k] = v1[k] = 0.0;
#pragma unroll 1
    for (int p = 0; p < D; ++p) {
      double sn, cn;
      LaneMath::sin_cos(x[p * LDX], &sn, &cn);
      const double rc = wu * cn;
      const double rs = wu * sn;
      const double* ur = sU + p * D;
#pragma unroll
      for (int k = 0; k < D - 1; ++k) {
        const double u = ur[k];
        v0[k] += u * rc;
        v1[k] += u * rs;
      }
    }
#pragma unroll
    for (int k = 0; k < D - 1; ++k) {
      const bool keep = k < K && fabs(sLam[k]) > kPinvAtol;
      v0[k] = keep ? v0[k] / wu : 0.0;
      v1[k] = keep ? v1[k] / wu : 0.0;
    }
    double sh[D];
#pragma unroll
    for (int k = 0; k < D; ++k) sh[k] = 0.0;
#pragma unroll 1
    for (int p = 0; p < D; ++p) {
      const double* ur = sU + p * D;
      double re = 0.0, im = 0.0;
#pragma unroll
      for (int k = 0; k < D - 1; ++k) {
        const double u = ur[k];
        re += u * v0[k];
        im += u * v1[k];
      }
      const double screen = LaneMath::arctan2(im, re);
#pragma unroll
      for (int k = 0; k < D; ++k) sh[k] += ur[k] * screen;
    }
#pragma unroll
    for (int k = 0; k < D; ++k) {
      const double lm = sLam[k];
      const bool keep = fabs(lm) > kPinvAtol;
      v0[k] = keep ? sh[k] / lm : 0.0;
      v1[k] = keep ? sh[k] : 0.0;
    }
    double* crow = coef + s * D;
#pragma unroll 1
    for (int p = 0; p < D; p += 2) {
      double wh[2] = {0.0, 0.0}, cw[2] = {0.0, 0.0};
#pragma unroll
      for (int q = 0; q < 2; ++q) {
        if (p + q < D) {
          const double* ur = sU + (p + q) * D;
#pragma unroll
          for (int r = 0; r < D; ++r) {
            const double u = ur[r];
            wh[q] += u * v0[r];
            cw[q] += u * v1[r];
          }
          x[(p + q) * LDX] = x[(p + q) * LDX] - cw[q];
        }
      }
      if (p + 1 < D) {
        __builtin_memcpy(crow + p, wh, 16);
      } else {
        crow[p] = wh[0];
      }
    }
  }

  lds_sync();
  store_rows<D, LDX>(resid + s0 * D, X, n_elem, __ballot(fitted));
  lds_sync();

  constexpr unsigned kFull = D == 32 ? ~0u : (1u << D) - 1u;
  unsigned um = kFull;
  bool alive = run;
  for (int it = 0; it < niter; ++it) {
    if (__ballot(alive) == 0ull) break;
    if (alive && it > 0) {
      const int n_unfl = __popc(um);
      double o = order;
      if (o > n_unfl - 1) o = n_unfl - 1;
      if (adjust_order) {
        double r[3];
        tree_sum3<D>(r, [&](int p, double(&v)[3]) {
          const bool unfl = (um >> p) & 1u;
          double sn = 0.0, cn = 0.0;
          if (unfl) LaneMath::sin_cos(x[p * LDX], &sn, &cn);
          const double ww = unfl ? wu : 0.0;
          v[0] = ww;
          v[1] = sn * sn * ww;
          v[2] = cn * cn * ww;
        });
        const double m1 = r[1] / r[0];
        const double m2 = r[2] / r[0];
        const double redchi2 = (1.0 - hypot(m1, m2)) * r[0] / (n_unfl - o);
        OrderWalk walk;
        double moved = o;
        if (!walk.template step<LaneMath>(0, redchi2, n_unfl, station_order, moved)) {
          defer = it;
          alive = false;
        }
      }
      if (alive) order = o;
    }
    if (alive && it + 1 < niter) {
      const auto wrapped = [&](int p) {
        double r = LaneMath::mod(x[p * LDX], 2.0 * M_PI);
        if (r < -M_PI) r += 2.0 * M_PI;
        if (r > M_PI) r -= 2.0 * M_PI;
        return r;
      };
      double t[3];
      tree_sum3<D>(t, [&](int p, double(&v)[3]) {
        const double r = wrapped(p);
        const bool inc = ((um >> p) & 1u) && !isnan(r);
        double sn = 0.0, cn = 0.0;
        if (inc) LaneMath::sin_cos(r, &sn, &cn);
        v[0] = inc ? 1.0 : 0.0;
        v[1] = sn;
        v[2] = cn;
      });
      const double ms = t[1] / t[0];
      const double mc = t[2] / t[0];
      const double stdv = sqrt(-2.0 * LaneMath::ln(hypot(ms, mc)));
      const double thr = nsigma * stdv;
      unsigned outl = 0u;
#pragma unroll 1
      for (int p = 0; p < D; ++p)
        if (fabs(wrapped(p)) > thr) outl |= 1u << p;
      if (outl) {
        um &= ~outl;
        int np = -2;
        if (um != 0u) {
          np = table_insert(keys, cap, (unsigned long long)um);
          if (np == -3) atomicOr(counters + kCntError, kErrTableFull);
        }
        pos[s] = np;
        if (um == 0u) alive = false;
      }
    }
  }

  lds_sync();
  const bool lost = fitted && um != kFull;
  if (lost) {
#pragma unroll 1
    for (int p = 0; p < D; ++p) x[p * LDX] = ((um >> p) & 1u) ? wu : 0.0;
  }
  lds_sync();
  store_rows<D, LDX>(w_out + s0 * D, X, n_elem, __ballot(lost));
  if (fitted) order_out[s] = (int32_t)order;
  const int dat = number_fresh(defer >= 0, counters + kCntList);
  if (defer >= 0) {
    cls[s] = kClassFast;
    list[dat] = list_entry(s, defer);
  }
  const unsigned long long nd = __ballot(defer >= 0);
  if (l == 0 && nd != 0ull) atomicAdd(counters + kCntLaneDeferred, __popcll(nd));
}

template <int D>
static void launch_lane(sf_ctx* ctx, const sf_fit_params* p, const RefSpec& r,
                        int64_t S, int A, const double* phase, double* coef,
                        double* resid, float* w_out, int32_t* order_out) {
  hipLaunchKernelGGL(kl_fit_lane_kernel<D>, dim3((unsigned)((S + 63) / 64)), dim3(64), 0,
                     ctx->stream, p->niter, S, A, phase, r.refph, r.sub, ctx->d_u,
                     ctx->d_eig, ctx->d_st_order, ctx->d_class, ctx->d_pos, ctx->d_keys,
                     (int)ctx->d_keys.size(), ctx->d_counters, ctx->d_list, p->nsigma,
                     p->adjust_order, coef, resid, w_out, order_out);
}

int launch_fit_lane(sf_ctx* ctx, const sf_fit_params* p, const RefSpec& r,
                    int64_t S, int A, const double* phase, double* coef,
                    double* resid, float* w_out, int32_t* order_out) {
  const int64_t per_block = 4 * 64 * kGroups;
  hipLaunchKernelGGL(kl_lane_list_kernel, dim3((unsigned)((S + per_block - 1) / per_block)),
                     dim3(256), 0, ctx->stream, ctx->d_class, S, ctx->d_counters,
                     ctx->d_list);
  SF_HIP(hipGetLastError());
#define SF_LANE_CASE(d)                                                        \
  case d:                                                                      \
    launch_lane<d>(ctx, p, r, S, A, phase, coef, resid, w_out, order_out);     \
    break;
  switch (ctx->D) {
    SF_LANE_CASE(3) SF_LANE_CASE(4) SF_LANE_CASE(5) SF_LANE_CASE(6)
    SF_LANE_CASE(7) SF_LANE_CASE(8) SF_LANE_CASE(9) SF_LANE_CASE(10)
    SF_LANE_CASE(11) SF_LANE_CASE(12) SF_LANE_CASE(13) SF_LANE_CASE(14)
    SF_LANE_CASE(15) SF_LANE_CASE(16) SF_LANE_CASE(17) SF_LANE_CASE(18)
    SF_LANE_CASE(19) SF_LANE_CASE(20) SF_LANE_CASE(21) SF_LANE_CASE(22)
    SF_LANE_CASE(23)
    default:
      set_error("sf_kl_fit: no lane kernel for this number of directions");
      return SF_EINVAL;
  }
#undef SF_LANE_CASE
  static_assert(kLaneMinD == 3 && kLaneMaxD == 23, "the cases above");
  SF_HIP(hipGetLastError());
  return SF_OK;
}

}
```

### ska-sdp-screen-fitting_amd/csrc/kl_fit_pool.h

```cpp
#pragma once

#include <hip/hip_runtime.h>

#include <algorithm>

#include "kl_fit_masks.h"
#include "kl_fit_steps.h"
#include "sf_internal.h"

namespace sf {

__device__ int table_find(const unsigned long long* keys, int cap,
                          unsigned long long key) {
  int h = (int)(mix64(key) & (unsigned long long)(cap - 1));
  for (int probe = 0; probe < cap; ++probe) {
    const unsigned long long k = keys[h];
    if (k == key) return h;
    if (k == kEmptyKey) return -1;
    h = (h + 1) & (cap - 1);
  }
  return -1;
}

__global__ __launch_bounds__(256) void kl_assign_kernel(
    const unsigned long long* __restrict__ keys, int cap, int* __restrict__ ids,
    unsigned long long* __restrict__ pool_mask, int pool_cap,
    int* __restrict__ counters, int D) {
  int lvl = 0;
  for (int i = blockIdx.x * blockDim.x + threadIdx.x; wave_in_table(i, cap);
       i += gridDim.x * blockDim.x) {
    const unsigned long long k = i < cap ? keys[i] : kEmptyKey;
    const int id = number_fresh(k != kEmptyKey && ids[i] < 0, counters + kCntIds);
    if (id < 0) continue;
    ids[i] = id;
    if (id < pool_cap) pool_mask[id] = k;
    lvl = max(lvl, D - __popcll(k));
  }
  for (int o = 32; o > 0; o >>= 1) lvl = max(lvl, __shfl_xor(lvl, o));
  if (lane() == 0 && lvl > 0) atomicMax(counters + kCntMaxLevel, lvl);
}

__host__ __device__ inline int subset_ld(int D) { return odd_ld(D > 1 ? D - 1 : 1); }
__host__ __device__ inline int subset_rows(int D) { return D > 1 ? D - 1 : 1; }
constexpr int kEigWavesDefault = 3;
template <int NW>
__global__ __launch_bounds__(64 * NW) void kl_subset_eig_kernel(
    const double* __restrict__ g_c, int D,
    const unsigned long long* __restrict__ pool_mask, int pool_cap,
    int* __restrict__ counters, double* __restrict__ pool,
    const uint8_t* __restrict__ done) {
  extern __shared__ double smem[];
  const int ld = subset_ld(D);
  double* a = smem;
  double* v = a + subset_rows(D) * ld;
  double2* cs = reinterpret_cast<double2*>(v + subset_rows(D) * ld);
  int2* pr = reinterpret_cast<int2*>(cs + 64);
  int* perm = reinterpret_cast<int*>(pr + 96);
  int* idx = perm + 64;
  const int first = counters[kCntPassStart];
  const int last = min(counters[kCntIds], pool_cap);
  const int l = lane();
  const bool w0 = threadIdx.x < 64;
  for (int id = first + blockIdx.x; id < last; id += gridDim.x) {
    if (done && done[id] == 0) continue;
    const unsigned long long m = pool_mask[id];
    const bool in = (l < D) && ((m >> l) & 1ull);
    const int n = __popcll(m);
    if (n >= D) {
      if (threadIdx.x == 0) atomicOr(counters + kCntError, kErrFullMaskInPool);
      continue;
    }
    if (w0 && in) idx[Group<1>::rank(m)] = l;
    __syncthreads();
    if (w0 && l < n) {
      const int r = idx[l];
      for (int q = 0; q < n; ++q) a[l * ld + q] = g_c[r * D + idx[q]];
    }
    __syncthreads();
    wg_jacobi<NW>(a, v, cs, pr, n, ld, kJacobiMaxSweeps);
    __syncthreads();
    if (w0) eig_order(Group<1>{}, a, n, ld, perm);
    double* e = pool + (size_t)id * (D * D + D);
    if (w0 && l < n) {
      for (int r = 0; r < n; ++r) e[l * D + r] = v[l * ld + perm[r]];
      const int pr = perm[l];
      e[D * D + l] = a[pr * ld + pr];
    }
    __syncthreads();
  }
}

__device__ __forceinline__ void load_ascending(const double* src, const double* eig,
                                               int stride, int m, double* U, int ld,
                                               double* lam, int* perm) {
#pragma clang fp contract(off)
  const int l = lane();
  if (l < m) perm[order_rank<AscendingValue>(m, l, [&](int k) { return eig[k]; })] = l;
  lds_sync();
  if (l < m) lam[l] = eig[perm[l]];
  for (int e = l; e < m * m; e += 64) {
    const int p = e / m, c = e % m;
    U[p * ld + c] = src[p * stride + perm[c]];
  }
}

__global__ __launch_bounds__(64) void kl_subset_secular_kernel(
    const double* __restrict__ g_u, const double* __restrict__ g_eig, int D,
    const unsigned long long* __restrict__ pool_mask, int pool_cap,
    int* __restrict__ counters, double* __restrict__ pool,
    uint8_t* __restrict__ status, const unsigned long long* __restrict__ keys,
    const int* __restrict__ ids, int table_cap, int level) {
#pragma clang fp contract(off)
  extern __shared__ double smem[];
  const int ld = odd_ld(D);
  double* U = smem;
  double* W = U + D * ld;
  double* lam = W + D * ld;
  double* lz = lam + 64;
  double* zh = lz + 64;
  double* tau = zh + 64;
  double* nlam = tau + 64;
  int* ndi = reinterpret_cast<int*>(nlam + 64);
  int* orig = ndi + 64;
  int* src = orig + 64;
  int* perm = src + 64;
  const int l = lane();
  const int first = counters[kCntPassStart];
  const int last = min(counters[kCntIds], pool_cap);
  constexpr double kEps = 2.220446049250313e-16;
  for (int id = first + blockIdx.x; id < last; id += gridDim.x) {
    const unsigned long long msk = pool_mask[id];
    const int n = __popcll(msk);
    if (level > 0 && D - n != level) continue;
    if (n >= D) {
      if (l == 0) status[id] = 1;
      continue;
    }
    const unsigned long long full = full_mask(D);
    unsigned long long anc = full;
    int aid = -1;
    if (level > 0) {
      unsigned long long a = msk;
      for (;;) {
        const unsigned long long fl = full & ~a;
        a |= fl & (~fl + 1ull);
        if (a == full) break;
        const int h = table_find(keys, table_cap, a);
        const int pid = h >= 0 ? ids[h] : -1;
        if (pid >= 0 && pid < pool_cap && status[pid] == 0) {
          anc = a;
          aid = pid;
          break;
        }
      }
    }
    int m = __popcll(anc);
    if (aid < 0) {
      load_ascending(g_u, g_eig, D, m, U, ld, lam, perm);
    } else {
      const double* ea = pool + (size_t)aid * (D * D + D);
      load_ascending(ea, ea + D * D, D, m, U, ld, lam, perm);
    }
    lds_sync();
    bool ok = true;
    for (int f = D - 1; f >= 0 && ok; --f) {
      if ((msk >> f) & 1ull) continue;
      if (!((anc >> f) & 1ull)) continue;
      const int j = f;
      const double z = l < m ? U[j * ld + l] : 0.0;
      const double zmax = wave_max(fabs(z));
      const double lmax = wave_max(l < m ? fabs(lam[l]) : 0.0);
      const bool nd = l < m && fabs(z) > 1e-14 * zmax;
      const unsigned long long ndm = __ballot(nd);
      const int nn = __popcll(ndm);
      const int kk = Group<1>::rank(ndm);
      if (nd) {
        ndi[kk] = l;
        lz[kk] = lam[l];
        zh[kk] = z;
      }
      lds_sync();
      const bool close = l + 1 < nn && lz[l + 1] - lz[l] <= 1e-12 * lmax;
      if (__ballot(close) != 0ull) {
        ok = false;
        break;
      }
      double t = 0.0;
      int o = 0;
      bool conv = true;
      if (l + 1 < nn) {
        const double lo = lz[l], hi = lz[l + 1];
        const double mid = lo + 0.5 * (hi - lo);
        double fm = 0.0;
#pragma unroll 4
        for (int k = 0; k < nn; ++k) {
          const double zk = zh[k];
          const double x = lz[k] - mid;
          double q = __builtin_amdgcn_rcp(x);
          q = q * (2.0 - x * q);
          fm += zk * zk * q;
        }
        double a, b;
        if (fm >= 0.0) {
          o = l;
          a = 0.0;
          b = mid - lo;
        } else {
          o = l + 1;
          a = mid - hi;
          b = 0.0;
        }
        const double lo_ = lz[o];
        const double zo = zh[o];
        const double zo2 = zo * zo;
        t = 0.5 * (a + b);
        conv = false;
        for (int it = 0; it < 64; ++it) {
          double rest = 0.0, drest = 0.0;
#pragma unroll 4
          for (int k = 0; k < nn; ++k) {
            const double zk = zh[k];
            const double x = (lz[k] - lo_) - t;
            double q = __builtin_amdgcn_rcp(x);
            q = q * (2.0 - x * q);
            q = k == o ? 0.0 : q;
            const double zq = zk * zk * q;
            rest += zq;
            drest += zq * q;
          }
          const double fv = rest - zo2 / t;
          if (fv == 0.0) {
            conv = true;
            break;
          }
          if (fv < 0.0) a = t; else b = t;
          double tn = t - (t * rest - zo2) / (rest + t * drest);
          if (fabs(tn - t) <= 4.0 * kEps * fabs(t)) {
            t = tn;
            conv = true;
            break;
          }
          if (!(tn > a && tn < b)) tn = 0.5 * (a + b);
          t = tn;
          if (!(b - a > 4.0 * kEps * fmax(fabs(a), fabs(b)))) {
            conv = true;
            break;
          }
        }
        tau[l] = t;
        orig[l] = o;
      }
      if (__ballot(!conv) != 0ull) {
        ok = false;
        break;
      }
      lds_sync();
      double zn = 0.0;
      if (l < nn) {
        const double lk = lz[l];
        double pr = 1.0;
#pragma unroll 4
        for (int r = 0; r + 1 < nn; ++r) {
          const int kp = r < l ? r : r + 1;
          pr *= ((lz[orig[r]] - lk) + tau[r]) / (lz[kp] - lk);
        }
        zn = sqrt(fabs(pr));
        if (zh[l] < 0.0) zn = -zn;
      }
      lds_sync();
      if (l < nn) zh[l] = zn;
      lds_sync();
      if (l + 1 < nn) {
        const double ol = lz[o];
        double nrm = 0.0;
#pragma unroll 4
        for (int k = 0; k < nn; ++k) {
          const double w = zh[k] / ((lz[k] - ol) - t);
          W[k * ld + l] = w;
          nrm += w * w;
        }
        const double inv = 1.0 / sqrt(nrm);
        for (int k = 0; k < nn; ++k) W[k * ld + l] *= inv;
      }
      const int dk = l - kk;
      if (l + 1 < nn) {
        nlam[l] = lz[o] + t;
        src[l] = l;
      }
      if (l < m && !nd) {
        nlam[nn - 1 + dk] = lam[l];
        src[nn - 1 + dk] = -1 - l;
      }
      lds_sync();
      if (l < m) {
        const bool dense = nn == m;
        int r = 0;
        for (; r + 4 < nn; r += 4) {
          double y0 = 0.0, y1 = 0.0, y2 = 0.0, y3 = 0.0;
#pragma unroll 2
          for (int k = 0; k < nn; ++k) {
            const double u = U[l * ld + (dense ? k : ndi[k])];
            const double* wk = W + k * ld + r;
            y0 += u * wk[0];
            y1 += u * wk[1];
            y2 += u * wk[2];
            y3 += u * wk[3];
          }
          lds_sync();
          W[l * ld + r] = y0;
          W[l * ld + r + 1] = y1;
          W[l * ld + r + 2] = y2;
          W[l * ld + r + 3] = y3;
        }
        for (; r + 1 < nn; ++r) {
          double y = 0.0;
          for (int k = 0; k < nn; ++k) y += U[l * ld + (dense ? k : ndi[k])] * W[k * ld + r];
          lds_sync();
          W[l * ld + r] = y;
        }
        for (int c = 0; c < m - nn; ++c) {
          const int sc = src[nn - 1 + c];
          W[l * ld + nn - 1 + c] = U[l * ld + (-1 - sc)];
        }
      }
      const int m1 = m - 1;
      if (l < m1) {
        const double v = nlam[l];
        int r2 = 0;
#pragma unroll 4
        for (int k = 0; k < m1; ++k) {
          r2 += ranks_before<AscendingValue>(nlam[k], k, v, l);
        }
        perm[r2] = l;
      }
      lds_sync();
      if (l < m && l != j) {
        const int pn = l < j ? l : l - 1;
        for (int c = 0; c < m1; ++c) U[pn * ld + c] = W[l * ld + perm[c]];
      }
      lds_sync();
      if (l < m1) lam[l] = nlam[perm[l]];
      if (l < m1) {
        double nr = 0.0;
#pragma unroll 4
        for (int r = 0; r < m1; ++r) {
          const double y = U[r * ld + l];
          nr += y * y;
        }
        tau[l] = sqrt(nr);
      }
      lds_sync();
      if (l < m1)
        for (int c = 0; c < m1; ++c) U[l * ld + c] = U[l * ld + c] / tau[c];
      lds_sync();
      m = m1;
    }
    if (!ok) {
      if (l == 0) status[id] = 1;
      continue;
    }
    if (l < m) perm[order_rank<DescendingAbs>(m, l, [&](int k) { return lam[k]; })] = l;
    lds_sync();
    double* e = pool + (size_t)id * (D * D + D);
    if (l < m) {
      for (int r = 0; r < m; ++r) e[l * D + r] = U[l * ld + perm[r]];
      e[D * D + l] = lam[perm[l]];
    }
    if (l == 0) status[id] = 0;
    lds_sync();
  }
}

static int ensure_pool(sf_ctx* ctx, size_t need) {
  const size_t entry = (size_t)ctx->D * ctx->D + ctx->D;
  if (ctx->pool_D != ctx->D) {
    ctx->d_pool.reset();
    ctx->d_pool_mask.reset();
    ctx->pool_D = ctx->D;
  }
  size_t cap = ctx->d_pool_mask.size() ? ctx->d_pool_mask.size() : 1024;
  while (cap < need) cap *= 2;
  SF_TRY(ctx->d_pool.reserve_keep(cap * entry, kFitAlloc));
  return ctx->d_pool_mask.reserve_keep(cap, kFitAlloc);
}

__global__ __launch_bounds__(256) void kl_fill_mask_kernel(
    const unsigned long long* __restrict__ keys, const int* __restrict__ ids,
    int cap, unsigned long long* __restrict__ pool_mask, int lo) {
  const int i = blockIdx.x * blockDim.x + threadIdx.x;
  if (i >= cap) return;
  if (keys[i] != kEmptyKey && ids[i] >= lo) pool_mask[ids[i]] = keys[i];
}

constexpr int kAncestorMinMasks = 8192;

static int number_and_decompose(sf_ctx* ctx, int* n_slow, int* n_nonuniform) {
  SF_HIP(hipMemcpyAsync(ctx->d_counters + kCntPassStart, ctx->d_counters + kCntIds,
                        sizeof(int), hipMemcpyDeviceToDevice, ctx->stream));
  SF_HIP(hipMemsetAsync(ctx->d_counters + kCntMaxLevel, 0, sizeof(int), ctx->stream));
  const int cap = (int)ctx->d_keys.size();
  const int old_cap = (int)ctx->d_pool_mask.size();
  hipLaunchKernelGGL(kl_assign_kernel, dim3(std::min((cap + 255) / 256, 8192)), dim3(256), 0,
                     ctx->stream, ctx->d_keys, cap, ctx->d_ids,
                     ctx->d_pool_mask, old_cap, ctx->d_counters, ctx->D);
  SF_HIP(hipGetLastError());
  int cnt[kCntMaxLevel + 1];
  SF_HIP(hipMemcpyAsync(cnt, ctx->d_counters, sizeof(cnt), hipMemcpyDeviceToHost,
                        ctx->stream));
  SF_HIP(hipStreamSynchronize(ctx->stream));
  *n_slow = cnt[kCntSlow];
  *n_nonuniform = cnt[kCntNonUniform];
  if (cnt[kCntIds] > old_cap) {
    SF_TRY(ensure_pool(ctx, (size_t)cnt[kCntIds]));
    hipLaunchKernelGGL(kl_fill_mask_kernel, dim3((cap + 255) / 256), dim3(256),
                       0, ctx->stream, ctx->d_keys, ctx->d_ids, cap,
                       ctx->d_pool_mask, old_cap);
    SF_HIP(hipGetLastError());
  }
  const int n_new = cnt[kCntIds] - cnt[kCntPassStart];
  const uint8_t* done = nullptr;
  if (n_new > 0 && ctx->fit_subset_deletion && ctx->D <= 64) {
    SF_TRY(ctx->d_pool_status.reserve_keep(ctx->d_pool_mask.size(),
                                           kFitAlloc));
    SF_HIP(hipMemsetAsync(ctx->d_pool_status + cnt[kCntPassStart], 1, (size_t)n_new, ctx->stream));
    const int D = ctx->D;
    const int ldd = odd_ld(D);
    const size_t shm = (size_t)2 * D * ldd * sizeof(double) + 6 * 64 * sizeof(double) +
                       4 * 64 * sizeof(int);
    SF_TRY(allow_lds(kl_subset_secular_kernel, shm));
    const int blocks = n_new < 16384 ? n_new : 16384;
    const bool anc = ctx->fit_subset_deletion == 3 ||
                     (ctx->fit_subset_deletion == 1 && n_new >= kAncestorMinMasks);
    const int levels = anc ? cnt[kCntMaxLevel] : 0;
    for (int lv = levels > 0 ? 1 : 0; lv <= levels; ++lv) {
      hipLaunchKernelGGL(kl_subset_secular_kernel, dim3(blocks), dim3(64), shm, ctx->stream,
                         ctx->d_u, ctx->d_eig, D, ctx->d_pool_mask, (int)ctx->d_pool_mask.size(),
                         ctx->d_counters, ctx->d_pool, ctx->d_pool_status, ctx->d_keys,
                         ctx->d_ids, cap, lv);
      SF_HIP(hipGetLastError());
    }
    done = ctx->d_pool_status;
  }
  if (n_new > 0) {
    const int D = ctx->D;
    const size_t shm = (size_t)2 * subset_rows(D) * subset_ld(D) * sizeof(double) +
                       64 * sizeof(double2) + 96 * sizeof(int2) +
                       128 * sizeof(int);
    const int blocks = n_new < 8192 ? n_new : 8192;
    const int nw = ctx->fit_eig_waves > 0 ? ctx->fit_eig_waves : kEigWavesDefault;
    decltype(&kl_subset_eig_kernel<1>) const eig[4] = {
        kl_subset_eig_kernel<1>, kl_subset_eig_kernel<2>, kl_subset_eig_kernel<3>,
        kl_subset_eig_kernel<4>};
    SF_TRY(allow_lds(eig[nw - 1], shm));
    hipLaunchKernelGGL(eig[nw - 1], dim3(blocks), dim3(64 * nw), shm, ctx->stream,
                       ctx->d_c, D, ctx->d_pool_mask, (int)ctx->d_pool_mask.size(),
                       ctx->d_counters, ctx->d_pool, done);
    SF_HIP(hipGetLastError());
  }
  return SF_OK;
}

}
```

### ska-sdp-screen-fitting_amd/csrc/sf_internal.h

```cpp
#pragma once

#include <hip/hip_runtime.h>

#include <cstdint>
#include <string>
#include <utility>
#include <vector>

#include "screenfit.h"

namespace sf {

void set_error(const std::string& msg);

#define SF_HIP(call)                                                        \
  do {                                                                      \
    hipError_t e_ = (call);                                                 \
    if (e_ != hipSuccess) {                                                 \
      ::sf::set_error(std::string(#call) + ": " + hipGetErrorString(e_));   \
      return SF_EIO;                                                        \
    }                                                                       \
  } while (0)

#define SF_REQUIRE(cond, code, msg) \
  do {                              \
    if (!(cond)) {                  \
      ::sf::set_error(msg);         \
      return (code);                \
    }                               \
  } while (0)

#define SF_TRY(x)                  \
  do {                             \
    int rc_ = (x);                 \
    if (rc_ != SF_OK) return rc_;  \
  } while (0)

template <typename T>
class DevBuf {
 public:
  DevBuf() = default;
  DevBuf(const DevBuf&) = delete;
  DevBuf& operator=(const DevBuf&) = delete;
  ~DevBuf() { reset(); }

  operator T*() const { return p_; }
  T* get() const { return p_; }
  size_t size() const { return n_; }

  void reset() {
    if (p_) (void)hipFree(p_);
    p_ = nullptr;
    n_ = 0;
  }
  void swap(DevBuf& o) {
    std::swap(p_, o.p_);
    std::swap(n_, o.n_);
  }

  int reserve(size_t need, const char* what) {
    if (n_ >= need) return SF_OK;
    reset();
    if (hipMalloc(reinterpret_cast<void**>(&p_), need * sizeof(T)) != hipSuccess) {
      p_ = nullptr;
      set_error(what);
      return SF_ENOMEM;
    }
    n_ = need;
    return SF_OK;
  }

  int reserve_keep(size_t need, const char* what) {
    if (n_ >= need) return SF_OK;
    DevBuf q;
    SF_TRY(q.reserve(need, what));
    if (n_ > 0 && hipMemcpy(q.p_, p_, n_ * sizeof(T), hipMemcpyDeviceToDevice) != hipSuccess) {
      set_error(std::string(what) + " (copy of the old contents)");
      return SF_EIO;
    }
    swap(q);
    return SF_OK;
  }

 private:
  T* p_ = nullptr;
  size_t n_ = 0;
};

template <typename T, typename U>
int reserve_pair(DevBuf<T>& p, size_t np, DevBuf<U>& q, size_t nq, const char* what) {
  if (p.size() >= np && q.size() >= nq) return SF_OK;
  p.reset();
  q.reset();
  SF_TRY(p.reserve(np, what));
  return q.reserve(nq, what);
}

constexpr const char* kFitAlloc = "hipMalloc failed (fit scratch)";

template <typename K>
int allow_lds(K* kernel, size_t shm) {
  if (shm > 64 * 1024)
    SF_HIP(hipFuncSetAttribute(reinterpret_cast<const void*>(kernel),
                               hipFuncAttributeMaxDynamicSharedMemorySize, (int)shm));
  return SF_OK;
}

enum FitCounter {
  kCntIds = 0,
  kCntWideDecomp = 0,
  kCntPassStart = 1,
  kCntSlow = 2,
  kCntError = 3,
  kCntNonUniform = 4,
  kCntMaxLevel = 5,
  kCntWideMasks = 6,
  kCntLaneDeferred = 7,
  kCntLane = 8,
  kCntList = 9,
};
constexpr int kFitCounters = 12;
enum FitError {
  kErrLookupMiss = 1,
  kErrTableFull = 2,
  kErrLeanNonUniform = 4,
  kErrFullMaskInPool = 8,
};

constexpr int kTiles = 4;
constexpr int kWavePix = 16 * kTiles;
constexpr int kEvalWaves = 4;
constexpr int kBlockPix = kWavePix * kEvalWaves;

constexpr int kDigits = 6;

}

struct sf_ctx {
  int device = 0;
  hipStream_t stream = nullptr;
  int D = 0;
  int has_basis = 0;
  int wide = 0;
  double r0 = 100.0;
  double beta = 5.0 / 3.0;
  sf::DevBuf<double> d_pp;
  sf::DevBuf<double> d_c;
  sf::DevBuf<double> d_pinv;
  sf::DevBuf<double> d_u;
  sf::DevBuf<double> d_eig;
  sf::DevBuf<double> d_wide_ws;
  int wide_cache = 1;
  int wide_pool_mb = 0;
  int wide_pool_max = 0;
  sf::DevBuf<unsigned long long> d_wkeys;
  sf::DevBuf<int> d_wslot;
  sf::DevBuf<unsigned long long> d_wtab;
  sf::DevBuf<int> d_wtab_id;
  sf::DevBuf<unsigned long long> d_wpool_mask;
  sf::DevBuf<double> d_wpool;
  int wide_pool_n = 0;
  int nx = 0, ny = 0;
  int64_t n_pix = 0;
  int64_t n_pix_blocks = 0;
  int ksteps = 0;
  sf::DevBuf<double> d_cfrag;
  double rev_thr = 0.0;
  sf::DevBuf<int8_t> d_cdig;
  int dig_ok = 0;
  int eval_int = -1;
  int eval_wg_waves = 0;
  sf::DevBuf<int8_t> d_kdig;
  sf::DevBuf<uint8_t> d_kflag;
  hipEvent_t kdig_read = nullptr;
  double h_pp[3 * SF_MAX_EVAL_DIR] = {};
  int n_points = 0;
  int pt_tiles = 0;
  int pt_ks_pad = 0;
  int pt_cus = 0;
  sf::DevBuf<double> d_pxy;
  sf::DevBuf<double> d_pfrag;
  int tec_F = 0;
  int tec_F_tec = 0;
  std::vector<int> tec_used;
  std::vector<int> tec_off;
  sf::DevBuf<double> d_tec_ch;
  sf::DevBuf<uint8_t> d_skip;
  sf::DevBuf<int> d_st_order;
  sf::DevBuf<unsigned long long> d_keys;
  sf::DevBuf<int> d_ids;
  sf::DevBuf<unsigned long long> d_pool_mask;
  sf::DevBuf<double> d_pool;
  int fit_eig_waves = 0;
  int fit_subset_deletion = 1;
  sf::DevBuf<uint8_t> d_pool_status;
  int pool_D = 0;
  sf::DevBuf<int> d_pos;
  sf::DevBuf<uint8_t> d_class;
  sf::DevBuf<long long> d_list;
  sf::DevBuf<double> d_sigma;
  sf::DevBuf<int> d_counters;
  sf::DevBuf<double> d_scratch;
  sf::DevBuf<float> d_wscratch;
  sf::DevBuf<int32_t> d_oscratch;
  sf::DevBuf<double> d_gw;
  double gw_sigma = -1.0;
  sf::DevBuf<float> d_trash;
  sf::DevBuf<float> d_smooth;
  sf::DevBuf<float> d_tess_tab;
  int force_general = 0;
  int eval_kernel = SF_EVAL_KERNEL_AUTO;
  int64_t eval_max_blocks = 0;
  int eval_ks_pad = 0;
  int eval_sleep = 0;
  int eval_xcd_map = -1;
  int eval_groups = 0;
  int eval_bands = 0;
  int tess_slots = 0;
  int tess_waves = 0;
  int tess_tile = 0;
  int tess_box = -1;
  int fit_pack = 1;
  int fit_lean = 1;
  int fit_lane = 1;
};

namespace sf {
constexpr int kEvalMaxKS = 15;
constexpr int kEvalWideMaxKS = SF_MAX_EVAL_DIR / 4;
inline bool eval_int_applies(const sf_ctx* ctx, bool gain, unsigned flags,
                             bool out_aligned16) {
  return !gain && ctx->dig_ok && ctx->d_cdig && ctx->eval_int != 0 &&
         (flags & SF_EVAL_FAST_SINCOS) && ctx->n_pix % 4 == 0 && out_aligned16 &&
         ctx->ksteps >= 12 && ctx->ksteps <= kEvalMaxKS;
}

struct RefSpec {
  int sub = -1;
  const double* refph = nullptr;
  int skip = -1;
};
RefSpec ref_spec(const sf_fit_params* p, int A);
int launch_skip(sf_ctx* ctx, const double* phase, const float* weight, int T,
                int F, int A, const RefSpec& r);
int launch_fit_general(sf_ctx* ctx, const double* phase, const float* weight,
                       int T, int F, int A, const sf_fit_params* p,
                       const RefSpec& r, double* coef, double* resid,
                       float* w_out, int32_t* order_out);
int launch_basis(sf_ctx* ctx);
int launch_block_sigma(sf_ctx* ctx, int T, int F, int A, const double* phase,
                       const RefSpec& r, int screen_type, const double* resid,
                       const float* w_out);
int fit_buffers(sf_ctx* ctx, int64_t S, int F, int A, double** resid,
                float** w_out, int32_t** order_out);
int launch_basis_wide(sf_ctx* ctx);
int launch_fit_wide(sf_ctx* ctx, const double* phase, const float* weight,
                    int T, int F, int A, const sf_fit_params* p, double* coef,
                    double* resid, float* w_out, int32_t* order_out);
int read_fit_pool_wide(sf_ctx* ctx, uint64_t* masks, double* entries, int k);
int launch_cpix(sf_ctx* ctx, const double* d_x, const double* d_y);
int launch_cdig(sf_ctx* ctx, const double* d_x, const double* d_y, int* d_bad);
int launch_fit(sf_ctx* ctx, const double* phase, const float* weight, int T,
               int F, int A, const sf_fit_params* p, double* coef,
               double* resid, float* w_out, int32_t* order_out);
int pick_eval_kernel(const sf_ctx* ctx, bool gain, unsigned flags,
                     bool out_aligned16);
int launch_eval(sf_ctx* ctx, const double* coef, const double* cxx,
                const double* cyy, int64_t S, float* out, int64_t ring,
                unsigned flags, unsigned* sums);
int launch_eval_wide(sf_ctx* ctx, const double* coef, const double* cxx,
                     const double* cyy, int64_t S, float* out, int64_t ring,
                     unsigned flags, unsigned* sums);
int launch_eval_pol(sf_ctx* ctx, const double* ph_xx, const double* ph_yy,
                    const double* amp_xx, const double* amp_yy, int64_t S, float* out,
                    int64_t ring, unsigned flags);
int launch_eval_values(sf_ctx* ctx, const double* coef, int64_t S, float* out,
                       int64_t ring, unsigned flags);
int launch_eval_tec(sf_ctx* ctx, const double* tec, const double* phase, int64_t T,
                    int A, float* out, unsigned flags);
int points_ks_pad(int D);
int points_tiles(int P);
int launch_points_cpix(sf_ctx* ctx);
int launch_eval_points(sf_ctx* ctx, const double* coef, const double* cxx,
                       const double* cyy, int64_t S, float* planes, unsigned flags);
int launch_eval_point_values(sf_ctx* ctx, const double* coef, int64_t S,
                             double* values);
int launch_tess(sf_ctx* ctx, const int32_t* labels, int nx, int ny,
                const double* phase, const double* phase_yy, const double* amp_xx,
                const double* amp_yy, int D, int64_t S, float* out,
                int64_t ring, const double* d_w, int R, unsigned flags);
int launch_tess_tile(sf_ctx* ctx, const int32_t* labels, int nx, int ny,
                const double* phase, const double* phase_yy, const double* amp_xx,
                const double* amp_yy, int D, int64_t S, float* out,
                int64_t ring, const double* d_w, int R, unsigned flags);
int launch_smooth(sf_ctx* ctx, float* cube, int nx, int ny, int64_t n_img,
                  const double* d_w, int R, unsigned flags);
constexpr int kTessMaxR = 24;
}
```

### ska-sdp-screen-fitting_amd/ska_sdp_screen_fitting_amd/_lib.py

```python

import contextlib
import ctypes
import os
import threading

import numpy as np

_HERE = os.path.dirname(os.path.abspath(__file__))
LIB_PATH = os.environ.get("SCREENFIT_LIB", os.path.join(_HERE, "libscreenfit.so"))

SF_SCREEN_PHASE = 0
SF_SCREEN_TEC = 1
SF_SCREEN_AMPLITUDE = 2
SF_EVAL_NAN_SCRUB = 1
SF_EVAL_FAST_SINCOS = 1 << 8
SF_EVAL_NT_STORES = 1 << 9
SF_EVAL_BIG_ENDIAN = 1 << 10
SF_MAX_DIR = 60
SF_MAX_FIT_DIR = 128
SF_MAX_EVAL_DIR = 128
SF_MAX_POINTS = 4096
SF_MAX_TEC_FREQ = 4096
SF_OPT_FIT_GENERAL = 1
SF_OPT_EVAL_KERNEL = 2
SF_OPT_EVAL_MAX_BLOCKS = 3
SF_OPT_FIT_PACK = 4
SF_OPT_EVAL_KS_PAD = 5
SF_OPT_EVAL_SLEEP = 6
SF_OPT_EVAL_XCD_MAP = 7
SF_OPT_EVAL_GROUPS = 8
SF_OPT_EVAL_BANDS = 9
SF_OPT_FIT_LEAN = 10
SF_OPT_TESS_SLOTS = 11
SF_OPT_TESS_WAVES = 12
SF_OPT_TESS_TILE = 13
SF_OPT_TESS_BOX = 14
SF_OPT_EVAL_INT = 15
SF_OPT_EVAL_WG_WAVES = 16
SF_OPT_FIT_EIG_WAVES = 17
SF_OPT_FIT_SUBSET_DELETION = 18
SF_OPT_FIT_WIDE_CACHE = 19
SF_OPT_FIT_WIDE_POOL_MB = 20
SF_OPT_FIT_WIDE_POOL_MAX = 21
SF_OPT_FIT_LANE = 22
SF_EVAL_KERNEL_AUTO = 0
SF_EVAL_KERNEL_TILE = 1
SF_EVAL_KERNEL_LDS4 = 2
SF_EVAL_KERNEL_LDS8 = 3
SF_EVAL_KERNEL_LDS16 = 4
SF_EVAL_KERNEL_LDS8H = 5
SF_EVAL_KERNEL_LDS16H = 6
SF_EVAL_KERNEL_TILE3 = 7
SF_EVAL_KERNEL_SHB = 8
SF_EVAL_KERNEL_WIDE = 9
EVAL_KERNEL_NAMES = {SF_EVAL_KERNEL_TILE: "kl_eval_kernel",
                     SF_EVAL_KERNEL_LDS4: "kl_eval_lds_kernel<4 waves>",
                     SF_EVAL_KERNEL_LDS8: "kl_eval_lds_kernel<8 waves>",
                     SF_EVAL_KERNEL_LDS16: "kl_eval_lds_kernel<16 waves>",
                     SF_EVAL_KERNEL_LDS8H: "kl_eval_lds_kernel<8 waves, 2 tiles>",
                     SF_EVAL_KERNEL_LDS16H: "kl_eval_lds_kernel<16 waves, 2 tiles>",
                     SF_EVAL_KERNEL_TILE3: "kl_eval_kernel<3 waves/SIMD>",
                     SF_EVAL_KERNEL_SHB: "kl_eval_kernel<Cpix in LDS>",
                     SF_EVAL_KERNEL_WIDE: "kl_eval_wide_kernel"}

EXPORTED = (
    "sf_version", "sf_last_error", "sf_create", "sf_destroy", "sf_set_stream",
    "sf_synchronize", "sf_set_option", "sf_get_eval_kernel", "sf_get_eval_contraction", "sf_alloc", "sf_free", "sf_copy_h2d", "sf_copy_d2h",
    "sf_set_basis", "sf_set_basis_wide", "sf_set_piercepoints", "sf_get_basis", "sf_kl_fit", "sf_get_fit_stats", "sf_get_fit_lane_stats", "sf_get_fit_pool",
    "sf_get_fit_pool_wide",
    "sf_stream_create", "sf_stream_destroy", "sf_device_cus",
    "sf_set_grid", "sf_kl_eval", "sf_kl_eval_gain", "sf_kl_eval_sums",
    "sf_tess_fill", "sf_smooth",
    "sf_set_points", "sf_kl_eval_points", "sf_kl_eval_point_values",
    "sf_kl_eval_values",
    "sf_set_tec_freqs", "sf_kl_eval_tec",
    "sf_kl_eval_pol", "sf_tess_fill_pol",
)


_identity = {}


def library_identity(path=None):
    import hashlib
    p = os.path.realpath(path or LIB_PATH)
    if p not in _identity:
        h = hashlib.sha256()
        with open(p, "rb") as fh:
            for blk in iter(lambda: fh.read(1 << 20), b""):
                h.update(blk)
        _identity[p] = {"sha16": h.hexdigest()[:16], "bytes": os.path.getsize(p)}
    return dict(_identity[p])


class ScreenFitError(RuntimeError):
    """Raised for any failure of the HIP library (including its absence)."""


class FitParams(ctypes.Structure):
    _fields_ = [("screen_type", ctypes.c_int), ("niter", ctypes.c_int),
                ("nsigma", ctypes.c_double), ("adjust_order", ctypes.c_int),
                ("ref_ant", ctypes.c_int), ("ant_offset", ctypes.c_int),
                ("ref_phase", ctypes.c_void_p)]


_lib = None
_lib_lock = threading.Lock()


def load_library(path=None):
    global _lib
    with _lib_lock:
        if _lib is not None and path is None:
            return _lib
        p = path or LIB_PATH
        if not os.path.exists(p):
            raise ScreenFitError(
                f"libscreenfit.so not found at {p}: build it with "
                "`make -C ska-sdp-screen-fitting_amd/csrc` (or "
                "__graft_entry__.build()); there is no CPU fallback")
        lib = ctypes.CDLL(p)
        vp, ip, c_int, c_dbl = (ctypes.c_void_p, ctypes.POINTER(ctypes.c_int),
                                ctypes.c_int, ctypes.c_double)
        i64 = ctypes.c_int64
        sig = {
            "sf_version": ([], ctypes.c_char_p),
            "sf_last_error": ([], ctypes.c_char_p),
            "sf_create": ([c_int, ctypes.POINTER(vp)], c_int),
            "sf_destroy": ([vp], c_int),
            "sf_set_stream": ([vp, vp], c_int),
            "sf_synchronize": ([vp], c_int),
            "sf_set_option": ([vp, c_int, c_int], c_int),
            "sf_get_eval_kernel": ([vp, c_int, ctypes.c_uint, ip], c_int),
            "sf_get_eval_contraction": ([vp, c_int, ctypes.c_uint, ip], c_int),
            "sf_alloc": ([vp, ctypes.c_size_t, ctypes.POINTER(vp)], c_int),
            "sf_free": ([vp, vp], c_int),
            "sf_copy_h2d": ([vp, vp, vp, ctypes.c_size_t], c_int),
            "sf_copy_d2h": ([vp, vp, vp, ctypes.c_size_t], c_int),
            "sf_set_basis": ([vp, vp, c_int, c_dbl, c_dbl], c_int),
            "sf_set_basis_wide": ([vp, vp, c_int, c_dbl, c_dbl], c_int),
            "sf_set_piercepoints": ([vp, vp, c_int, c_dbl, c_dbl], c_int),
            "sf_get_basis": ([vp, vp, vp, vp, vp], c_int),
            "sf_kl_fit": ([vp, vp, vp, c_int, c_int, c_int, ip,
                           ctypes.POINTER(FitParams), vp, vp, vp, vp], c_int),
            "sf_get_fit_stats": ([vp, ip, ip], c_int),
            "sf_get_fit_lane_stats": ([vp, ctypes.POINTER(i64), ctypes.POINTER(i64)], c_int),
            "sf_get_fit_pool": ([vp, vp, vp, c_int, ip], c_int),
            "sf_get_fit_pool_wide": ([vp, vp, vp, c_int, ip], c_int),
            "sf_set_grid": ([vp, vp, c_int, vp, c_int], c_int),
            "sf_kl_eval": ([vp, vp, i64, vp, i64, ctypes.c_uint], c_int),
            "sf_stream_create": ([vp, ctypes.POINTER(c_int), c_int,
                                  ctypes.POINTER(vp)], c_int),
            "sf_stream_destroy": ([vp, vp], c_int),
            "sf_device_cus": ([vp, ctypes.POINTER(c_int)], c_int),
            "sf_kl_eval_gain": ([vp, vp, vp, vp, i64, vp, i64, ctypes.c_uint],
                                c_int),
            "sf_kl_eval_sums": ([vp, vp, vp, vp, i64, vp, i64, ctypes.c_uint, vp],
                                c_int),
            "sf_tess_fill": ([vp, vp, c_int, c_int, vp, vp, vp, c_int, i64, vp,
                              i64, c_dbl, ctypes.c_uint], c_int),
            "sf_smooth": ([vp, vp, c_int, c_int, i64, c_dbl, ctypes.c_uint], c_int),
            "sf_set_points": ([vp, vp, c_int], c_int),
            "sf_kl_eval_points": ([vp, vp, vp, vp, i64, vp, ctypes.c_uint], c_int),
            "sf_kl_eval_point_values": ([vp, vp, i64, vp], c_int),
            "sf_kl_eval_values": ([vp, vp, i64, vp, i64, ctypes.c_uint], c_int),
            "sf_set_tec_freqs": ([vp, vp, vp, c_int, c_int], c_int),
            "sf_kl_eval_tec": ([vp, vp, vp, i64, c_int, vp, ctypes.c_uint], c_int),
            "sf_kl_eval_pol": ([vp, vp, vp, vp, vp, i64, vp, i64, ctypes.c_uint],
                               c_int),
            "sf_tess_fill_pol": ([vp, vp, c_int, c_int, vp, vp, vp, vp, c_int, i64,
                                  vp, i64, c_dbl, ctypes.c_uint], c_int),
        }
        for name, (args, res) in sig.items():
            fn = getattr(lib, name)
            fn.argtypes = args
            fn.restype = res
        if path is None:
            _lib = lib
        return lib


def _check(rc, what):
    if rc != 0:
        msg = load_library().sf_last_error().decode(errors="replace")
        raise ScreenFitError(f"{what} failed ({rc}): {msg}")


_TORCH_DTYPES = {np.float64: "torch.float64", np.float32: "torch.float32",
                 np.int32: "torch.int32", np.int64: "torch.int64"}


def _dev(x, dtype, numel, name, device=None):
    if x is None or isinstance(x, int):
        return x
    if not hasattr(x, "data_ptr"):
        raise TypeError(f"{name}: expected a device tensor, got {type(x).__name__}")
    if not x.is_cuda:
        raise ValueError(f"{name}: must be a device (cuda) tensor")
    if device is not None and x.device.index != device:
        raise ValueError(f"{name}: on cuda:{x.device.index}, the context is on "
                         f"cuda:{device}")
    if str(x.dtype) != _TORCH_DTYPES[dtype]:
        raise TypeError(f"{name}: dtype {x.dtype}, expected {_TORCH_DTYPES[dtype]}")
    if not x.is_contiguous():
        raise ValueError(f"{name}: must be contiguous")
    if x.numel() < numel:
        raise ValueError(f"{name}: {x.numel()} elements, the call needs {numel}")
    return x.data_ptr()


class Context:

    def __init__(self, device=0):
        self.lib = load_library()
        self.device = device
        h = ctypes.c_void_p()
        _check(self.lib.sf_create(device, ctypes.byref(h)), "sf_create")
        self.h = h
        self.D = 0
        self.grid = None
        self.points = 0
        self.tec_freqs = None
        self.options = {}

    def close(self):
        if self.h:
            self.lib.sf_destroy(self.h)
            self.h = None

    def __del__(self):
        try:
            self.close()
        except Exception:
            pass

    def _dev(self, x, dtype, numel, name):
        return _dev(x, dtype, numel, name, self.device)

    def set_stream(self, stream_handle):
        _check(self.lib.sf_set_stream(self.h, stream_handle), "sf_set_stream")

    def set_option(self, option, value):
        _check(self.lib.sf_set_option(self.h, int(option), int(value)),
               "sf_set_option")
        self.options[int(option)] = int(value)

    def eval_kernel(self, flags, gain=False):
        k = ctypes.c_int()
        _check(self.lib.sf_get_eval_kernel(self.h, int(bool(gain)), int(flags),
                                           ctypes.byref(k)), "sf_get_eval_kernel")
        name = EVAL_KERNEL_NAMES[k.value]
        if (self.options.get(SF_OPT_EVAL_WG_WAVES, 0) == 8
                and k.value in (SF_EVAL_KERNEL_TILE, SF_EVAL_KERNEL_TILE3)
                and self.eval_contraction(flags, gain) == "i8-digits"):
            name += " (8-wave workgroups)"
        return name

    def eval_contraction(self, flags, gain=False):
        k = ctypes.c_int()
        _check(self.lib.sf_get_eval_contraction(self.h, int(bool(gain)), int(flags),
                                                ctypes.byref(k)), "sf_get_eval_contraction")
        return "i8-digits" if k.value == 1 else "f64"

    def synchronize(self):
        _check(self.lib.sf_synchronize(self.h), "sf_synchronize")

    def set_basis(self, pp, r0=100.0, beta=5.0 / 3.0):
        pp = np.ascontiguousarray(pp, dtype=np.float64)
        assert pp.ndim == 2 and pp.shape[1] == 3
        _check(self.lib.sf_set_basis(self.h, pp.ctypes.data, pp.shape[0],
                                     float(r0), float(beta)), "sf_set_basis")
        self.D = pp.shape[0]
        self.grid = None
        self.points = 0

    def set_basis_wide(self, pp, r0=100.0, beta=5.0 / 3.0):
        pp = np.ascontiguousarray(pp, dtype=np.float64)
        assert pp.ndim == 2 and pp.shape[1] == 3
        self.D = 0
        self.grid = None
        self.points = 0
        _check(self.lib.sf_set_basis_wide(self.h, pp.ctypes.data, pp.shape[0],
                                          float(r0), float(beta)),
               "sf_set_basis_wide")
        self.D = pp.shape[0]

    def set_piercepoints(self, pp, r0=100.0, beta=5.0 / 3.0):
        pp = np.ascontiguousarray(pp, dtype=np.float64)
        assert pp.ndim == 2 and pp.shape[1] == 3
        self.D = 0
        self.grid = None
        self.points = 0
        _check(self.lib.sf_set_piercepoints(self.h, pp.ctypes.data, pp.shape[0],
                                            float(r0), float(beta)),
               "sf_set_piercepoints")
        self.D = pp.shape[0]

    def get_basis(self):
        D = self.D
        c, pinv, u = (np.empty((D, D)) for _ in range(3))
        eig = np.empty(D)
        _check(self.lib.sf_get_basis(self.h, c.ctypes.data, pinv.ctypes.data,
                                     u.ctypes.data, eig.ctypes.data),
               "sf_get_basis")
        return c, pinv, u, eig

    def fit(self, phase, weight, T, F, A, station_order, screen_type=0,
            niter=2, nsigma=5.0, adjust_order=True, ref_ant=-1, coef=None,
            resid=None, w_out=None, order_out=None, ant_offset=0,
            ref_phase=None):
        so = np.ascontiguousarray(station_order, dtype=np.int32)
        if so.shape != (A,):
            raise ValueError(f"station_order: shape {so.shape}, expected ({A},)")
        n = int(T) * int(F) * int(A) * self.D
        prm = FitParams(int(screen_type), int(niter), float(nsigma),
                        int(bool(adjust_order)), int(ref_ant), int(ant_offset),
                        self._dev(ref_phase, np.float64, int(T) * int(F) * self.D,
                             "ref_phase"))
        _check(self.lib.sf_kl_fit(
            self.h, self._dev(phase, np.float64, n, "phase"),
            self._dev(weight, np.float32, n, "weight"), int(T), int(F), int(A),
            so.ctypes.data_as(ctypes.POINTER(ctypes.c_int)),
            ctypes.byref(prm), self._dev(coef, np.float64, n, "coef"),
            self._dev(resid, np.float64, n, "resid"),
            self._dev(w_out, np.float32, n, "w_out"),
            self._dev(order_out, np.int32, n // max(self.D, 1), "order_out")),
            "sf_kl_fit")

    def fit_stats(self):
        nm, ng = ctypes.c_int(), ctypes.c_int()
        _check(self.lib.sf_get_fit_stats(self.h, ctypes.byref(nm), ctypes.byref(ng)),
               "sf_get_fit_stats")
        return {"n_masks": nm.value, "n_general": ng.value}

    def fit_lane_stats(self):
        nl, nd = ctypes.c_int64(), ctypes.c_int64()
        _check(self.lib.sf_get_fit_lane_stats(self.h, ctypes.byref(nl), ctypes.byref(nd)),
               "sf_get_fit_lane_stats")
        return {"n_lane": nl.value, "n_deferred": nd.value}

    def fit_pool(self):
        n = ctypes.c_int(0)
        _check(self.lib.sf_get_fit_pool(self.h, None, None, 0, ctypes.byref(n)),
               "sf_get_fit_pool")
        D = self.D
        masks = np.zeros(n.value, np.uint64)
        ent = np.zeros((n.value, D * D + D))
        if n.value:
            _check(self.lib.sf_get_fit_pool(self.h, masks.ctypes.data, ent.ctypes.data,
                                            n.value, ctypes.byref(n)), "sf_get_fit_pool")
        order = np.argsort(masks, kind="stable")
        masks, ent = masks[order], ent[order]
        for k, m in enumerate(masks):
            n = bin(int(m)).count("1")
            u = ent[k, :D * D].reshape(D, D)
            u[n:, :] = 0.0
            u[:, n:] = 0.0
            ent[k, D * D + n:] = 0.0
        return masks, ent

    def fit_pool_wide(self):
        n = ctypes.c_int(0)
        _check(self.lib.sf_get_fit_pool_wide(self.h, None, None, 0, ctypes.byref(n)),
               "sf_get_fit_pool_wide")
        D = self.D
        masks = np.zeros((n.value, 2), np.uint64)
        ent = np.zeros((n.value, D * D + D))
        if n.value:
            _check(self.lib.sf_get_fit_pool_wide(self.h, masks.ctypes.data,
                                                 ent.ctypes.data, n.value,
                                                 ctypes.byref(n)),
                   "sf_get_fit_pool_wide")
        order = np.lexsort((masks[:, 0], masks[:, 1]))
        return masks[order], ent[order]

    def set_grid(self, x, y):
        x = np.ascontiguousarray(x, dtype=np.float64)
        y = np.ascontiguousarray(y, dtype=np.float64)
        _check(self.lib.sf_set_grid(self.h, x.ctypes.data, x.size,
                                    y.ctypes.data, y.size), "sf_set_grid")
        self.grid = (x.size, y.size)

    def _out_numel(self, S, ring):
        nx, ny = self.grid if self.grid else (0, 0)
        return min(int(S), ring) * 4 * nx * ny

    def eval(self, coef, S, out, ring_slots=None,
             flags=SF_EVAL_NAN_SCRUB | SF_EVAL_FAST_SINCOS | SF_EVAL_NT_STORES):
        ring = max(int(S if ring_slots is None else ring_slots), 1)
        _check(self.lib.sf_kl_eval(
            self.h, self._dev(coef, np.float64, int(S) * self.D, "coef"), int(S),
            self._dev(out, np.float32, self._out_numel(S, ring), "out"), ring,
            int(flags)), "sf_kl_eval")

    def eval_values(self, coef, S, out, ring_slots=None, flags=0):
        ring = max(int(S if ring_slots is None else ring_slots), 1)
        _check(self.lib.sf_kl_eval_values(
            self.h, self._dev(coef, np.float64, int(S) * self.D, "coef"), int(S),
            self._dev(out, np.float32, self._out_numel(S, ring) // 4, "out"), ring,
            int(flags)), "sf_kl_eval_values")

    def eval_pol(self, phase_xx, phase_yy, S, out, ring_slots=None, amp_xx=None,
                 amp_yy=None,
                 flags=SF_EVAL_NAN_SCRUB | SF_EVAL_FAST_SINCOS | SF_EVAL_NT_STORES):
        ring = max(int(S if ring_slots is None else ring_slots), 1)
        n = int(S) * self.D
        _check(self.lib.sf_kl_eval_pol(
            self.h, self._dev(phase_xx, np.float64, n, "phase_xx"),
            self._dev(phase_yy, np.float64, n, "phase_yy"),
            self._dev(amp_xx, np.float64, n, "amp_xx"),
            self._dev(amp_yy, np.float64, n, "amp_yy"), int(S),
            self._dev(out, np.float32, self._out_numel(S, ring), "out"), ring,
            int(flags)), "sf_kl_eval_pol")

    def set_tec_freqs(self, rad_per_tecu, tec_index=None, n_tec_freq=None):
        k = np.ascontiguousarray(rad_per_tecu, dtype=np.float64).reshape(-1)
        idx = None
        if tec_index is not None:
            idx = np.ascontiguousarray(tec_index, dtype=np.int32).reshape(-1)
            if idx.shape != k.shape:
                raise ValueError(f"tec_index: shape {idx.shape}, expected {k.shape}")
        if n_tec_freq is None:
            n_tec_freq = 1 if idx is None or idx.size == 0 else int(idx.max()) + 1
        _check(self.lib.sf_set_tec_freqs(
            self.h, k.ctypes.data, None if idx is None else idx.ctypes.data,
            k.size, int(n_tec_freq)), "sf_set_tec_freqs")
        self.tec_freqs = (int(k.size), int(n_tec_freq))

    def eval_tec(self, tec_coef, T, A, out, phase_coef=None,
                 flags=SF_EVAL_NAN_SCRUB | SF_EVAL_FAST_SINCOS | SF_EVAL_NT_STORES):
        F, F_tec = self.tec_freqs if self.tec_freqs else (0, 0)
        nx, ny = self.grid if self.grid else (0, 0)
        n = int(T) * F_tec * int(A) * self.D
        _check(self.lib.sf_kl_eval_tec(
            self.h, self._dev(tec_coef, np.float64, n, "tec_coef"),
            self._dev(phase_coef, np.float64, n, "phase_coef"), int(T), int(A),
            self._dev(out, np.float32, int(T) * F * int(A) * 4 * nx * ny, "out"),
            int(flags)), "sf_kl_eval_tec")

    def set_points(self, xy):
        xy = np.ascontiguousarray(xy, dtype=np.float64)
        if xy.ndim != 2 or xy.shape[1] != 2:
            raise ValueError(f"xy: shape {xy.shape}, expected (P, 2)")
        self.points = 0
        _check(self.lib.sf_set_points(self.h, xy.ctypes.data, xy.shape[0]),
               "sf_set_points")
        self.points = xy.shape[0]

    def eval_points(self, coef, S, planes, coef_xx=None, coef_yy=None,
                    flags=SF_EVAL_NAN_SCRUB | SF_EVAL_FAST_SINCOS):
        n = int(S) * self.D
        _check(self.lib.sf_kl_eval_points(
            self.h, self._dev(coef, np.float64, n, "coef"),
            self._dev(coef_xx, np.float64, n, "coef_xx"),
            self._dev(coef_yy, np.float64, n, "coef_yy"), int(S),
            self._dev(planes, np.float32, int(S) * 4 * self.points, "planes"),
            int(flags)), "sf_kl_eval_points")

    def eval_point_values(self, coef, S, values):
        _check(self.lib.sf_kl_eval_point_values(
            self.h, self._dev(coef, np.float64, int(S) * self.D, "coef"), int(S),
            self._dev(values, np.float64, int(S) * self.points, "values")),
            "sf_kl_eval_point_values")

    def device_cus(self):
        n = ctypes.c_int(0)
        _check(self.lib.sf_device_cus(self.h, ctypes.byref(n)), "sf_device_cus")
        return n.value

    def stream_create(self, reserve_cus=()):
        arr = (ctypes.c_int * max(1, len(reserve_cus)))(*reserve_cus)
        out = ctypes.c_void_p()
        _check(self.lib.sf_stream_create(self.h, arr, len(reserve_cus),
                                         ctypes.byref(out)), "sf_stream_create")
        return out.value

    def stream_destroy(self, stream):
        _check(self.lib.sf_stream_destroy(self.h, ctypes.c_void_p(stream)),
               "sf_stream_destroy")

    def eval_gain(self, coef_ph, coef_xx, coef_yy, S, out, ring_slots=None,
                  flags=SF_EVAL_NAN_SCRUB | SF_EVAL_FAST_SINCOS | SF_EVAL_NT_STORES):
        ring = max(int(S if ring_slots is None else ring_slots), 1)
        n = int(S) * self.D
        _check(self.lib.sf_kl_eval_gain(
            self.h, self._dev(coef_ph, np.float64, n, "coef_ph"),
            self._dev(coef_xx, np.float64, n, "coef_xx"),
            self._dev(coef_yy, np.float64, n, "coef_yy"), int(S),
            self._dev(out, np.float32, self._out_numel(S, ring), "out"), ring,
            int(flags)), "sf_kl_eval_gain")

    def eval_sums(self, coef, S, out, sums, ring_slots=None, coef_xx=None,
                  coef_yy=None,
                  flags=SF_EVAL_NAN_SCRUB | SF_EVAL_FAST_SINCOS | SF_EVAL_NT_STORES):
        ring = max(int(S if ring_slots is None else ring_slots), 1)
        n = int(S) * self.D
        _check(self.lib.sf_kl_eval_sums(
            self.h, self._dev(coef, np.float64, n, "coef"),
            self._dev(coef_xx, np.float64, n, "coef_xx"),
            self._dev(coef_yy, np.float64, n, "coef_yy"), int(S),
            self._dev(out, np.float32, self._out_numel(S, ring), "out"), ring,
            int(flags), self._dev(sums, np.int32, int(S), "sums")), "sf_kl_eval_sums")

    def tess_fill(self, labels, nx, ny, phase, D, S, out, ring_slots=None,
                  amp_xx=None, amp_yy=None, smooth_pix=0.0,
                  flags=SF_EVAL_NAN_SCRUB, phase_yy=None):
        ring = max(int(S if ring_slots is None else ring_slots), 1)
        n = int(S) * int(D)
        if hasattr(labels, "min") and labels.numel():
            import weakref
            prev = getattr(self, "_labels_ok", None)
            key = (labels._version, int(D))
            if prev is None or prev[0]() is not labels or prev[1] != key:
                lo, hi = int(labels.min()), int(labels.max())
                if lo < 1 or hi > int(D):
                    raise ValueError(f"labels: values {lo}..{hi} outside 1..{D}")
                self._labels_ok = (weakref.ref(labels), key)
        _check(self.lib.sf_tess_fill_pol(
            self.h, self._dev(labels, np.int32, int(nx) * int(ny), "labels"),
            int(nx), int(ny), self._dev(phase, np.float64, n, "phase"),
            self._dev(phase_yy, np.float64, n, "phase_yy"),
            self._dev(amp_xx, np.float64, n, "amp_xx"),
            self._dev(amp_yy, np.float64, n, "amp_yy"), int(D), int(S),
            self._dev(out, np.float32, min(int(S), ring) * 4 * int(nx) * int(ny), "out"),
            ring, float(smooth_pix), int(flags)), "sf_tess_fill")


    def smooth(self, cube, nx, ny, n_img, smooth_pix, flags=0):
        _check(self.lib.sf_smooth(
            self.h, self._dev(cube, np.float32, int(n_img) * int(nx) * int(ny), "cube"),
            int(nx), int(ny), int(n_img), float(smooth_pix), int(flags)), "sf_smooth")


_contexts = {}
_ctx_lock = threading.Lock()


def get_context(device=0):
    with _ctx_lock:
        ctx = _contexts.get(device)
        if ctx is None:
            ctx = Context(device)
            _contexts[device] = ctx
    return ctx


_idle = {}
_IDLE_MAX = 4


@contextlib.contextmanager
def private_context(device=0):
    with _ctx_lock:
        idle = _idle.setdefault(device, [])
        ctx = idle.pop() if idle else None
    if ctx is None:
        ctx = Context(device)
    try:
        yield ctx
    finally:
        with _ctx_lock:
            keep = len(_idle[device]) < _IDLE_MAX
            if keep:
                _idle[device].append(ctx)
        if not keep:
            ctx.close()
```

Before: 6.289 million.

## Group fast-path slots by flag mask and fit them in per-mask lane kernel

Adds a masked lane-fit path that buckets fast-class slots by their pooled mask id using a count, prefix-scan and scatter sequence of kernels. Each bucket is then solved in waves of 64 rows that share one LDS-resident decomposition, so these slots skip the generic per-slot pass. The later-iteration logic is factored into a shared helper that writes through a row-index indirection. This adds three small kernels plus a single-block scan and extra buffers, and it is enabled by default when masks are uniform and the mask count fits in the bins.

```diff
diff --git a/include/screenfit.h b/include/screenfit.h
--- a/include/screenfit.h
+++ b/include/screenfit.h
@@ -71,6 +71,8 @@
 #define SF_OPT_FIT_WIDE_POOL_MB 20
 #define SF_OPT_FIT_WIDE_POOL_MAX 21
 #define SF_OPT_FIT_LANE 22
+#define SF_OPT_FIT_LANE_MASKED 23
+#define SF_OPT_FIT_LANE_MASK_MIN 24
 #define SF_EVAL_KERNEL_AUTO 0
 #define SF_EVAL_KERNEL_TILE 1
 #define SF_EVAL_KERNEL_LDS4 2
@@ -109,6 +111,8 @@
 int sf_get_fit_stats(sf_ctx* ctx, int* n_masks, int* n_general);
 
 int sf_get_fit_lane_stats(sf_ctx* ctx, int64_t* n_lane, int64_t* n_deferred);
+
+int sf_get_fit_lane_masked_stats(sf_ctx* ctx, int64_t* n_masked, int64_t* n_deferred);
 
 int sf_get_fit_pool(sf_ctx* ctx, uint64_t* masks_host, double* entries_host,
                     int max_masks, int* n_masks);
diff --git a/ska-sdp-screen-fitting_amd/csrc/capi.hip b/ska-sdp-screen-fitting_amd/csrc/capi.hip
--- a/ska-sdp-screen-fitting_amd/csrc/capi.hip
+++ b/ska-sdp-screen-fitting_amd/csrc/capi.hip
@@ -159,6 +159,13 @@
       return SF_OK;
     case SF_OPT_FIT_LANE:
       ctx->fit_lane = value != 0;
+      return SF_OK;
+    case SF_OPT_FIT_LANE_MASKED:
+      ctx->fit_lane_masked = value != 0;
+      return SF_OK;
+    case SF_OPT_FIT_LANE_MASK_MIN:
+      SF_REQUIRE(value >= 0, SF_EINVAL, "sf_set_option: mask minimum must be >= 0");
+      ctx->fit_lane_mask_min = value;
       return SF_OK;
     case SF_OPT_EVAL_KS_PAD:
       SF_REQUIRE(value >= 0 && value <= 3, SF_EINVAL,
@@ -468,6 +475,18 @@
   return SF_OK;
 }
 
+int sf_get_fit_lane_masked_stats(sf_ctx* ctx, int64_t* n_masked, int64_t* n_deferred) {
+  SF_REQUIRE(ctx, SF_EINVAL, "sf_get_fit_lane_masked_stats: NULL context");
+  int c[sf::kFitCounters] = {};
+  SF_HIP(hipSetDevice(ctx->device));
+  SF_HIP(hipStreamSynchronize(ctx->stream));
+  if (ctx->d_counters)
+    SF_HIP(hipMemcpy(c, ctx->d_counters, sizeof(c), hipMemcpyDeviceToHost));
+  if (n_masked) *n_masked = c[sf::kCntLaneMasked];
+  if (n_deferred) *n_deferred = c[sf::kCntLaneMaskedDeferred];
+  return SF_OK;
+}
+
 int sf_get_fit_pool(sf_ctx* ctx, uint64_t* masks_host, double* entries_host,
                     int max_masks, int* n_masks) {
   SF_REQUIRE(ctx && n_masks && max_masks >= 0, SF_EINVAL, "sf_get_fit_pool: bad argument");
diff --git a/ska-sdp-screen-fitting_amd/csrc/kl_fit_fast.hip b/ska-sdp-screen-fitting_amd/csrc/kl_fit_fast.hip
--- a/ska-sdp-screen-fitting_amd/csrc/kl_fit_fast.hip
+++ b/ska-sdp-screen-fitting_amd/csrc/kl_fit_fast.hip
@@ -619,10 +619,11 @@
 
   const bool block_flags = p->screen_type != SF_SCREEN_PHASE;
   for (int it = 0; it < p->niter; ++it) {
-    int n_slow = 0, n_nonuniform = 0;
-    SF_TRY(number_and_decompose(ctx, &n_slow, &n_nonuniform));
+    int n_slow = 0, n_nonuniform = 0, n_ids = 0;
+    SF_TRY(number_and_decompose(ctx, &n_slow, &n_nonuniform, &n_ids));
     if (it == 0 && lane_fit)
-      SF_TRY(launch_fit_lane(ctx, p, r, S, A, phase, coef, resid, w_out, order_out));
+      SF_TRY(launch_fit_lane(ctx, p, r, S, A, phase, coef, resid, w_out, order_out,
+                             n_ids, n_nonuniform));
     SF_TRY(launch_pass(ctx, false, it, p, r, S, F, A, phase, coef, resid, w_out,
                           order_out, n_nonuniform == 0, list));
     if (n_slow > 0)
diff --git a/ska-sdp-screen-fitting_amd/csrc/kl_fit_lane.h b/ska-sdp-screen-fitting_amd/csrc/kl_fit_lane.h
--- a/ska-sdp-screen-fitting_amd/csrc/kl_fit_lane.h
+++ b/ska-sdp-screen-fitting_amd/csrc/kl_fit_lane.h
@@ -10,6 +10,10 @@
 
 constexpr int kLaneMinD = 3;
 constexpr int kLaneMaxD = 23;
+
+constexpr int kMaskBins = 4096;
+constexpr int kLaneMaskedMaxD = 23;
+constexpr int kLaneMaskMin = 16;
 
 constexpr int kListPassShift = 56;
 __host__ __device__ inline long long list_entry(int64_t s, int first) {
@@ -30,6 +34,7 @@
 
 int launch_fit_lane(sf_ctx* ctx, const sf_fit_params* p, const RefSpec& r,
                     int64_t S, int A, const double* phase, double* coef,
-                    double* resid, float* w_out, int32_t* order_out);
+                    double* resid, float* w_out, int32_t* order_out, int n_ids,
+                    int n_nonuniform);
 
 }
diff --git a/ska-sdp-screen-fitting_amd/csrc/kl_fit_lane.hip b/ska-sdp-screen-fitting_amd/csrc/kl_fit_lane.hip
--- a/ska-sdp-screen-fitting_amd/csrc/kl_fit_lane.hip
+++ b/ska-sdp-screen-fitting_amd/csrc/kl_fit_lane.hip
@@ -54,13 +54,115 @@
   for (int k = 0; k < 3; ++k) out[k] = t5[k];
 }
 
-template <int D, int LDX, class T>
-__device__ __forceinline__ void store_rows(T* dst, const double* X, int n_elem,
-                                           unsigned long long rows) {
+template <int D, int LDX, class T, class Rows>
+__device__ __forceinline__ void store_rows(T* dst, const Rows& at, const double* X,
+                                           int n_elem, unsigned long long rows) {
   for (int e = lane(); e < n_elem; e += 64) {
     const int r = e / D, d = e % D;
-    if ((rows >> r) & 1ull) dst[e] = (T)X[d * LDX + r];
-  }
+    if ((rows >> r) & 1ull) dst[at.slot(r) * D + d] = (T)X[d * LDX + r];
+  }
+}
+
+struct ConsecutiveRows {
+  int64_t s0;
+  __device__ __forceinline__ int64_t slot(int r) const { return s0 + r; }
+};
+
+template <int D, int LDX, class Rows>
+__device__ __forceinline__ void lane_later_passes(
+    double* X, double* x, const Rows& rows, int n_elem, int64_t s, bool run, int defer,
+    unsigned um0, double wu, double station_order, double order, int niter,
+    int adjust_order, double nsigma, uint8_t* __restrict__ cls, int* __restrict__ pos,
+    unsigned long long* __restrict__ keys, int cap, int* __restrict__ counters,
+    int deferred_counter, long long* __restrict__ list, float* __restrict__ w_out,
+    int32_t* __restrict__ order_out) {
+  const int l = lane();
+  const bool fitted = run;
+  unsigned um = um0;
+  bool alive = run;
+  for (int it = 0; it < niter; ++it) {
+    if (__ballot(alive) == 0ull) break;
+    if (alive && it > 0) {
+      const int n_unfl = __popc(um);
+      double o = order;
+      if (o > n_unfl - 1) o = n_unfl - 1;
+      if (adjust_order) {
+        double r[3];
+        tree_sum3<D>(r, [&](int p, double(&v)[3]) {
+          const bool unfl = (um >> p) & 1u;
+          double sn = 0.0, cn = 0.0;
+          if (unfl) LaneMath::sin_cos(x[p * LDX], &sn, &cn);
+          const double ww = unfl ? wu : 0.0;
+          v[0] = ww;
+          v[1] = sn * sn * ww;
+          v[2] = cn * cn * ww;
+        });
+        const double m1 = r[1] / r[0];
+        const double m2 = r[2] / r[0];
+        const double redchi2 = (1.0 - hypot(m1, m2)) * r[0] / (n_unfl - o);
+        OrderWalk walk;
+        double moved = o;
+        if (!walk.template step<LaneMath>(0, redchi2, n_unfl, station_order, moved)) {
+          defer = it;
+          alive = false;
+        }
+      }
+      if (alive) order = o;
+    }
+    if (alive && it + 1 < niter) {
+      const auto wrapped = [&](int p) {
+        double r = LaneMath::mod(x[p * LDX], 2.0 * M_PI);
+        if (r < -M_PI) r += 2.0 * M_PI;
+        if (r > M_PI) r -= 2.0 * M_PI;
+        return r;
+      };
+      double t[3];
+      tree_sum3<D>(t, [&](int p, double(&v)[3]) {
+        const double r = wrapped(p);
+        const bool inc = ((um >> p) & 1u) && !isnan(r);
+        double sn = 0.0, cn = 0.0;
+        if (inc) LaneMath::sin_cos(r, &sn, &cn);
+        v[0] = inc ? 1.0 : 0.0;
+        v[1] = sn;
+        v[2] = cn;
+      });
+      const double ms = t[1] / t[0];
+      const double mc = t[2] / t[0];
+      const double stdv = sqrt(-2.0 * LaneMath::ln(hypot(ms, mc)));
+      const double thr = nsigma * stdv;
+      unsigned outl = 0u;
+#pragma unroll 1
+      for (int p = 0; p < D; ++p)
+        if (fabs(wrapped(p)) > thr) outl |= 1u << p;
+      if (outl) {
+        um &= ~outl;
+        int np = -2;
+        if (um != 0u) {
+          np = table_insert(keys, cap, (unsigned long long)um);
+          if (np == -3) atomicOr(counters + kCntError, kErrTableFull);
+        }
+        pos[s] = np;
+        if (um == 0u) alive = false;
+      }
+    }
+  }
+
+  lds_sync();
+  const bool lost = fitted && um != um0;
+  if (lost) {
+#pragma unroll 1
+    for (int p = 0; p < D; ++p) x[p * LDX] = ((um >> p) & 1u) ? wu : 0.0;
+  }
+  lds_sync();
+  store_rows<D, LDX>(w_out, rows, X, n_elem, __ballot(lost));
+  if (fitted) order_out[s] = (int32_t)order;
+  const int dat = number_fresh(defer >= 0, counters + kCntList);
+  if (defer >= 0) {
+    cls[s] = kClassFast;
+    list[dat] = list_entry(s, defer);
+  }
+  const unsigned long long nd = __ballot(defer >= 0);
+  if (l == 0 && nd != 0ull) atomicAdd(counters + deferred_counter, __popcll(nd));
 }
 
 constexpr int kGroups = 16;
@@ -222,95 +324,347 @@
   }
 
   lds_sync();
-  store_rows<D, LDX>(resid + s0 * D, X, n_elem, __ballot(fitted));
+  const ConsecutiveRows rows{s0};
+  store_rows<D, LDX>(resid, rows, X, n_elem, __ballot(fitted));
   lds_sync();
 
   constexpr unsigned kFull = D == 32 ? ~0u : (1u << D) - 1u;
-  unsigned um = kFull;
-  bool alive = run;
-  for (int it = 0; it < niter; ++it) {
-    if (__ballot(alive) == 0ull) break;
-    if (alive && it > 0) {
-      const int n_unfl = __popc(um);
-      double o = order;
-      if (o > n_unfl - 1) o = n_unfl - 1;
-      if (adjust_order) {
-        double r[3];
-        tree_sum3<D>(r, [&](int p, double(&v)[3]) {
-          const bool unfl = (um >> p) & 1u;
-          double sn = 0.0, cn = 0.0;
-          if (unfl) LaneMath::sin_cos(x[p * LDX], &sn, &cn);
-          const double ww = unfl ? wu : 0.0;
-          v[0] = ww;
-          v[1] = sn * sn * ww;
-          v[2] = cn * cn * ww;
-        });
-        const double m1 = r[1] / r[0];
-        const double m2 = r[2] / r[0];
-        const double redchi2 = (1.0 - hypot(m1, m2)) * r[0] / (n_unfl - o);
-        OrderWalk walk;
-        double moved = o;
-        if (!walk.template step<LaneMath>(0, redchi2, n_unfl, station_order, moved)) {
-          defer = it;
-          alive = false;
+  lane_later_passes<D, LDX>(X, x, rows, n_elem, s, run, defer, kFull, wu, station_order,
+                            order, niter, adjust_order, nsigma, cls, pos, keys, cap,
+                            counters, kCntLaneDeferred, list, w_out, order_out);
+}
+
+constexpr int kBinCursor = kMaskBins, kBinTotal = 2 * kMaskBins;
+constexpr int kBlockSlots = 4 * 64 * kGroups;
+
+__device__ __forceinline__ int fast_slot_id(const uint8_t* cls, const int* pos,
+                                            const int* ids, int64_t s, int64_t S,
+                                            int n_ids) {
+  if (s >= S || cls[s] != kClassFast) return -1;
+  const int p = pos[s];
+  if (p < 0) return -1;
+  const int id = ids[p];
+  return (unsigned)id < (unsigned)n_ids ? id : -1;
+}
+
+__global__ __launch_bounds__(256) void kl_mask_count_kernel(
+    const uint8_t* __restrict__ cls, const int* __restrict__ pos,
+    const int* __restrict__ ids, int64_t S, int n_ids, int* __restrict__ bins) {
+  __shared__ int hist[kMaskBins];
+  for (int b = threadIdx.x; b < n_ids; b += 256) hist[b] = 0;
+  __syncthreads();
+  const int64_t sb = (int64_t)blockIdx.x * kBlockSlots;
+  for (int i = threadIdx.x; i < kBlockSlots; i += 256) {
+    const int id = fast_slot_id(cls, pos, ids, sb + i, S, n_ids);
+    if (id >= 0) atomicAdd(&hist[id], 1);
+  }
+  __syncthreads();
+  for (int b = threadIdx.x; b < n_ids; b += 256)
+    if (hist[b] != 0) atomicAdd(bins + b, hist[b]);
+}
+
+__global__ __launch_bounds__(1024) void kl_mask_prefix_kernel(
+    const unsigned long long* __restrict__ pool_mask, int n_ids, int min_slots,
+    int* __restrict__ bins, long long* __restrict__ glist, int* __restrict__ counters) {
+  constexpr int kPer = kMaskBins / 1024;
+  __shared__ int part[1024];
+  __shared__ int n_masked;
+  const int t = threadIdx.x;
+  if (t == 0) n_masked = 0;
+  int cnt[kPer], len[kPer], sum = 0, masked = 0;
+#pragma unroll
+  for (int j = 0; j < kPer; ++j) {
+    const int b = kPer * t + j;
+    cnt[j] = b < n_ids ? bins[b] : 0;
+    const bool grouped = cnt[j] > 0 && cnt[j] >= min_slots && __popcll(pool_mask[b]) >= 3;
+    len[j] = grouped ? (cnt[j] + 63) & ~63 : 0;
+    sum += len[j];
+    masked += grouped ? cnt[j] : 0;
+  }
+  part[t] = sum;
+  __syncthreads();
+  for (int o = 1; o < 1024; o <<= 1) {
+    const int v = t >= o ? part[t - o] : 0;
+    __syncthreads();
+    part[t] += v;
+    __syncthreads();
+  }
+  if (masked != 0) atomicAdd(&n_masked, masked);
+  int off = part[t] - sum;
+#pragma unroll
+  for (int j = 0; j < kPer; ++j) {
+    const int b = kPer * t + j;
+    if (b >= n_ids) break;
+    bins[kBinCursor + b] = len[j] != 0 ? off : -1;
+    for (int i = off + cnt[j]; i < off + len[j]; ++i) glist[i] = -1;
+    off += len[j];
+  }
+  __syncthreads();
+  if (t == 1023) bins[kBinTotal] = part[1023];
+  if (t == 0) counters[kCntLaneMasked] = n_masked;
+}
+
+__global__ __launch_bounds__(256) void kl_mask_scatter_kernel(
+    const uint8_t* __restrict__ cls, const int* __restrict__ pos,
+    const int* __restrict__ ids, int64_t S, int n_ids, int* __restrict__ bins,
+    int* __restrict__ counters, long long* __restrict__ list,
+    long long* __restrict__ glist) {
+  __shared__ int hist[kMaskBins];
+  for (int b = threadIdx.x; b < n_ids; b += 256) hist[b] = 0;
+  __syncthreads();
+  const int l = lane();
+  const int64_t sb = ((int64_t)blockIdx.x * 4 + threadIdx.x / 64) * (64 * kGroups);
+  int my_at[kGroups];
+  int my_id[kGroups];
+  int my_rank[kGroups];
+  int n_fast = 0, n_lane = 0;
+#pragma unroll
+  for (int g = 0; g < kGroups; ++g) {
+    const int64_t sg = sb + g * 64 + l;
+    const uint8_t c = sg < S ? cls[sg] : kClassSkipped;
+    int id = c == kClassFast ? fast_slot_id(cls, pos, ids, sg, S, n_ids) : -1;
+    if (id >= 0 && bins[kBinCursor + id] < 0) id = -1;
+    my_id[g] = id;
+    my_rank[g] = id >= 0 ? atomicAdd(&hist[id], 1) : 0;
+    const unsigned long long fast_rows = __ballot(c == kClassFast && id < 0);
+    my_at[g] = c == kClassFast && id < 0 ? n_fast + Group<1>::rank(fast_rows) : -1;
+    n_fast += __popcll(fast_rows);
+    n_lane += __popcll(__ballot(c == kClassLane));
+  }
+  unsigned long long old = 0ull;
+  if (l == 0 && (n_fast | n_lane) != 0)
+    old = atomicAdd(reinterpret_cast<unsigned long long*>(counters + kCntLane),
+                    (unsigned long long)n_lane | ((unsigned long long)n_fast << 32));
+  const int base = (int)(__shfl(old, 0) >> 32);
+  __syncthreads();
+  for (int b = threadIdx.x; b < n_ids; b += 256) {
+    const int h = hist[b];
+    if (h != 0) hist[b] = atomicAdd(bins + kBinCursor + b, h);
+  }
+  __syncthreads();
+#pragma unroll
+  for (int g = 0; g < kGroups; ++g) {
+    const int64_t sg = sb + g * 64 + l;
+    if (my_at[g] >= 0) list[base + my_at[g]] = list_entry(sg, 0);
+    if (my_id[g] >= 0) glist[hist[my_id[g]] + my_rank[g]] = sg;
+  }
+}
+
+struct ListedRows {
+  const long long* row_s;
+  __device__ __forceinline__ int64_t slot(int r) const { return row_s[r]; }
+};
+
+template <int D>
+__global__ __launch_bounds__(64, 2) void kl_fit_lane_masked_kernel(
+    int niter, int A, const double* __restrict__ phase,
+    const double* __restrict__ refph, int ref_sub,
+    const double* __restrict__ g_u, const double* __restrict__ g_c,
+    const double* __restrict__ g_eig, const int* __restrict__ st_order,
+    uint8_t* __restrict__ cls, int* __restrict__ pos, const int* __restrict__ ids,
+    unsigned long long* __restrict__ keys, int cap, const double* __restrict__ pool,
+    const unsigned long long* __restrict__ pool_mask, const int* __restrict__ bins,
+    int* __restrict__ counters, long long* __restrict__ list,
+    const long long* __restrict__ glist, double nsigma, int adjust_order,
+    double* __restrict__ coef, double* __restrict__ resid, float* __restrict__ w_out,
+    int32_t* __restrict__ order_out) {
+  constexpr int LDX = 65;
+  __shared__ double X[D * LDX];
+  __shared__ double Y[D * LDX];
+  __shared__ double sU[D * D + D];
+  __shared__ long long row_s[64];
+  __shared__ long long row_tf[64];
+  __shared__ int row_a[64];
+  const int l = lane();
+  const int64_t i0 = (int64_t)blockIdx.x * 64;
+  if (i0 >= bins[kBinTotal]) return;
+  const int64_t s = glist[i0 + l];
+  const bool mine = s >= 0;
+  const int id = __builtin_amdgcn_readfirstlane(mine ? ids[pos[s]] : 0);
+  const unsigned m0 = (unsigned)pool_mask[id];
+  const int n = __popc(m0);
+  const int a = mine ? (int)(s % A) : 0;
+  const double* sLam = sU + D * D;
+  {
+    const double* e = pool + (size_t)id * (D * D + D);
+    for (int i = l; i < D * D; i += 64) sU[i] = (i / D < n && i % D < n) ? e[i] : 0.0;
+    if (l < D) sU[D * D + l] = l < n ? e[D * D + l] : 0.0;
+  }
+  row_s[l] = s;
+  row_a[l] = a;
+  row_tf[l] = mine ? (long long)(s / A) : 0;
+  lds_sync();
+  for (int i = l; i < 64 * D; i += 64) {
+    const int r = i / D, d = i % D;
+    const int64_t sr = row_s[r];
+    double v = 0.0;
+    if (sr >= 0) {
+      v = phase[sr * D + d];
+      if (refph) v -= refph[row_tf[r] * D + d];
+      else if (ref_sub >= 0) v -= phase[(sr + (ref_sub - row_a[r])) * D + d];
+    }
+    X[d * LDX + r] = v;
+  }
+  lds_sync();
+  double* x = X + l;
+  double* y = Y + l;
+
+  bool run = mine;
+  int defer = -1;
+  if (run) {
+    bool finite = true;
+#pragma unroll 1
+    for (int d = 0; d < D; ++d) finite = finite && __builtin_isfinite(x[d * LDX]);
+    if (!finite) {
+      defer = 0;
+      run = false;
+    }
+  }
+  const double wu = mine ? (double)w_out[s * D + __builtin_ctz(m0)] : 1.0;
+  const double station_order = mine ? (double)st_order[a] : 0.0;
+  double order = station_order;
+
+  if (run) {
+    if (order > n - 1) order = n - 1;
+    const int K = (int)order;
+    double v0[D], v1[D];
+#pragma unroll
+    for (int k = 0; k < D; ++k) v0[k] = v1[k] = 0.0;
+    unsigned mm = m0;
+#pragma unroll 1
+    for (int p = 0; p < n; ++p) {
+      const int d = __builtin_ctz(mm);
+      mm &= mm - 1u;
+      double sn, cn;
+      LaneMath::sin_cos(x[d * LDX], &sn, &cn);
+      const double rc = wu * cn;
+      const double rs = wu * sn;
+      const double* ur = sU + p * D;
+#pragma unroll
+      for (int k = 0; k < D - 1; ++k) {
+        const double u = ur[k];
+        v0[k] += u * rc;
+        v1[k] += u * rs;
+      }
+    }
+#pragma unroll
+    for (int k = 0; k < D - 1; ++k) {
+      const bool keep = k < K && fabs(sLam[k]) > kPinvAtol;
+      v0[k] = keep ? v0[k] / wu : 0.0;
+      v1[k] = keep ? v1[k] / wu : 0.0;
+    }
+    double sh[D];
+#pragma unroll
+    for (int k = 0; k < D; ++k) sh[k] = 0.0;
+    mm = m0;
+#pragma unroll 1
+    for (int p = 0; p < n; ++p) {
+      const int d = __builtin_ctz(mm);
+      mm &= mm - 1u;
+      const double* ur = sU + p * D;
+      double re = 0.0, im = 0.0;
+#pragma unroll
+      for (int k = 0; k < D - 1; ++k) {
+        const double u = ur[k];
+        re += u * v0[k];
+        im += u * v1[k];
+      }
+      const double screen = LaneMath::arctan2(im, re);
+#pragma unroll
+      for (int k = 0; k < D; ++k) sh[k] += ur[k] * screen;
+      y[d * LDX] = screen;
+      x[d * LDX] = x[d * LDX] - screen;
+    }
+#pragma unroll
+    for (int k = 0; k < D; ++k) {
+      const double lm = sLam[k];
+      v0[k] = fabs(lm) > kPinvAtol ? sh[k] / lm : 0.0;
+    }
+    double sf[D];
+#pragma unroll
+    for (int f = 0; f < D; ++f) sf[f] = 0.0;
+    mm = m0;
+#pragma unroll 1
+    for (int p = 0; p < n; ++p) {
+      const int d = __builtin_ctz(mm);
+      mm &= mm - 1u;
+      const double* ur = sU + p * D;
+      double white = 0.0;
+#pragma unroll
+      for (int r = 0; r < D; ++r) white += ur[r] * v0[r];
+#pragma unroll
+      for (int f = 0; f < D; ++f)
+        if (!((m0 >> f) & 1u)) sf[f] += g_c[f * D + d] * white;
+    }
+#pragma unroll
+    for (int f = 0; f < D; ++f)
+      if (!((m0 >> f) & 1u)) {
+        y[f * LDX] = sf[f];
+        x[f * LDX] = x[f * LDX] - sf[f];
+      }
+  }
+
+  lds_sync();
+  for (int i = l; i < D * D; i += 64) sU[i] = g_u[i];
+  if (l < D) sU[D * D + l] = g_eig[l];
+  lds_sync();
+
+  if (run) {
+    double sh[D];
+#pragma unroll
+    for (int k = 0; k < D; ++k) sh[k] = 0.0;
+#pragma unroll 1
+    for (int p = 0; p < D; ++p) {
+      const double* ur = sU + p * D;
+      const double screen = y[p * LDX];
+#pragma unroll
+      for (int k = 0; k < D; ++k) sh[k] += ur[k] * screen;
+    }
+#pragma unroll
+    for (int k = 0; k < D; ++k) {
+      const double lm = sLam[k];
+      sh[k] = fabs(lm) > kPinvAtol ? sh[k] / lm : 0.0;
+    }
+    double* crow = coef + s * D;
+#pragma unroll 1
+    for (int p = 0; p < D; p += 2) {
+      double wh[2] = {0.0, 0.0};
+#pragma unroll
+      for (int q = 0; q < 2; ++q) {
+        if (p + q < D) {
+          const double* ur = sU + (p + q) * D;
+#pragma unroll
+          for (int r = 0; r < D; ++r) wh[q] += ur[r] * sh[r];
         }
       }
-      if (alive) order = o;
-    }
-    if (alive && it + 1 < niter) {
-      const auto wrapped = [&](int p) {
-        double r = LaneMath::mod(x[p * LDX], 2.0 * M_PI);
-        if (r < -M_PI) r += 2.0 * M_PI;
-        if (r > M_PI) r -= 2.0 * M_PI;
-        return r;
-      };
-      double t[3];
-      tree_sum3<D>(t, [&](int p, double(&v)[3]) {
-        const double r = wrapped(p);
-        const bool inc = ((um >> p) & 1u) && !isnan(r);
-        double sn = 0.0, cn = 0.0;
-        if (inc) LaneMath::sin_cos(r, &sn, &cn);
-        v[0] = inc ? 1.0 : 0.0;
-        v[1] = sn;
-        v[2] = cn;
-      });
-      const double ms = t[1] / t[0];
-      const double mc = t[2] / t[0];
-      const double stdv = sqrt(-2.0 * LaneMath::ln(hypot(ms, mc)));
-      const double thr = nsigma * stdv;
-      unsigned outl = 0u;
-#pragma unroll 1
-      for (int p = 0; p < D; ++p)
-        if (fabs(wrapped(p)) > thr) outl |= 1u << p;
-      if (outl) {
-        um &= ~outl;
-        int np = -2;
-        if (um != 0u) {
-          np = table_insert(keys, cap, (unsigned long long)um);
-          if (np == -3) atomicOr(counters + kCntError, kErrTableFull);
-        }
-        pos[s] = np;
-        if (um == 0u) alive = false;
-      }
-    }
-  }
-
-  lds_sync();
-  const bool lost = fitted && um != kFull;
-  if (lost) {
-#pragma unroll 1
-    for (int p = 0; p < D; ++p) x[p * LDX] = ((um >> p) & 1u) ? wu : 0.0;
-  }
-  lds_sync();
-  store_rows<D, LDX>(w_out + s0 * D, X, n_elem, __ballot(lost));
-  if (fitted) order_out[s] = (int32_t)order;
-  const int dat = number_fresh(defer >= 0, counters + kCntList);
-  if (defer >= 0) {
-    cls[s] = kClassFast;
-    list[dat] = list_entry(s, defer);
-  }
-  const unsigned long long nd = __ballot(defer >= 0);
-  if (l == 0 && nd != 0ull) atomicAdd(counters + kCntLaneDeferred, __popcll(nd));
+      if (p + 1 < D) {
+        __builtin_memcpy(crow + p, wh, 16);
+      } else {
+        crow[p] = wh[0];
+      }
+    }
+  }
+
+  lds_sync();
+  const ListedRows rows{row_s};
+  store_rows<D, LDX>(resid, rows, X, 64 * D, __ballot(run));
+  lds_sync();
+
+  lane_later_passes<D, LDX>(X, x, rows, 64 * D, s, run, defer, m0, wu, station_order,
+                            order, niter, adjust_order, nsigma, cls, pos, keys, cap,
+                            counters, kCntLaneMaskedDeferred, list, w_out, order_out);
+}
+
+template <int D>
+static void launch_lane_masked(sf_ctx* ctx, const sf_fit_params* p, const RefSpec& r,
+                               unsigned waves, int A, const double* phase, double* coef,
+                               double* resid, float* w_out, int32_t* order_out) {
+  hipLaunchKernelGGL(kl_fit_lane_masked_kernel<D>, dim3(waves), dim3(64), 0, ctx->stream,
+                     p->niter, A, phase, r.refph, r.sub, ctx->d_u, ctx->d_c, ctx->d_eig,
+                     ctx->d_st_order, ctx->d_class, ctx->d_pos, ctx->d_ids, ctx->d_keys,
+                     (int)ctx->d_keys.size(), ctx->d_pool, ctx->d_pool_mask,
+                     ctx->d_mask_bins, ctx->d_counters, ctx->d_list, ctx->d_glist,
+                     p->nsigma, p->adjust_order, coef, resid, w_out, order_out);
 }
 
 template <int D>
@@ -324,14 +678,56 @@
                      p->adjust_order, coef, resid, w_out, order_out);
 }
 
+static bool lane_masked_applies(const sf_ctx* ctx, int n_ids, int n_nonuniform) {
+  return ctx->fit_lane_masked && n_nonuniform == 0 && n_ids > 0 && n_ids <= kMaskBins &&
+         ctx->D >= kLaneMinD && ctx->D <= kLaneMaskedMaxD;
+}
+
 int launch_fit_lane(sf_ctx* ctx, const sf_fit_params* p, const RefSpec& r,
                     int64_t S, int A, const double* phase, double* coef,
-                    double* resid, float* w_out, int32_t* order_out) {
-  const int64_t per_block = 4 * 64 * kGroups;
-  hipLaunchKernelGGL(kl_lane_list_kernel, dim3((unsigned)((S + per_block - 1) / per_block)),
-                     dim3(256), 0, ctx->stream, ctx->d_class, S, ctx->d_counters,
-                     ctx->d_list);
+                    double* resid, float* w_out, int32_t* order_out, int n_ids,
+                    int n_nonuniform) {
+  const dim3 list_grid((unsigned)((S + kBlockSlots - 1) / kBlockSlots));
+  const bool masked = lane_masked_applies(ctx, n_ids, n_nonuniform);
+  if (masked) {
+    SF_TRY(ctx->d_mask_bins.reserve((size_t)kBinTotal + 1, kFitAlloc));
+    SF_TRY(ctx->d_glist.reserve((size_t)S + 64 * (size_t)kMaskBins, kFitAlloc));
+    SF_HIP(hipMemsetAsync(ctx->d_mask_bins, 0, kMaskBins * sizeof(int), ctx->stream));
+    hipLaunchKernelGGL(kl_mask_count_kernel, list_grid, dim3(256), 0, ctx->stream,
+                       ctx->d_class, ctx->d_pos, ctx->d_ids, S, n_ids, ctx->d_mask_bins);
+    const int min_slots = ctx->fit_lane_mask_min > 0 ? ctx->fit_lane_mask_min : kLaneMaskMin;
+    hipLaunchKernelGGL(kl_mask_prefix_kernel, dim3(1), dim3(1024), 0, ctx->stream,
+                       ctx->d_pool_mask, n_ids, min_slots, ctx->d_mask_bins, ctx->d_glist,
+                       ctx->d_counters);
+    hipLaunchKernelGGL(kl_mask_scatter_kernel, list_grid, dim3(256), 0, ctx->stream,
+                       ctx->d_class, ctx->d_pos, ctx->d_ids, S, n_ids, ctx->d_mask_bins,
+                       ctx->d_counters, ctx->d_list, ctx->d_glist);
+  } else {
+    hipLaunchKernelGGL(kl_lane_list_kernel, list_grid, dim3(256), 0, ctx->stream,
+                       ctx->d_class, S, ctx->d_counters, ctx->d_list);
+  }
   SF_HIP(hipGetLastError());
+  if (masked) {
+    const unsigned waves = (unsigned)(S / 64 + n_ids);
+#define SF_LANE_CASE(d)                                                                 \
+  case d:                                                                               \
+    launch_lane_masked<d>(ctx, p, r, waves, A, phase, coef, resid, w_out, order_out);   \
+    break;
+    switch (ctx->D) {
+      SF_LANE_CASE(3) SF_LANE_CASE(4) SF_LANE_CASE(5) SF_LANE_CASE(6)
+      SF_LANE_CASE(7) SF_LANE_CASE(8) SF_LANE_CASE(9) SF_LANE_CASE(10)
+      SF_LANE_CASE(11) SF_LANE_CASE(12) SF_LANE_CASE(13) SF_LANE_CASE(14)
+      SF_LANE_CASE(15) SF_LANE_CASE(16) SF_LANE_CASE(17) SF_LANE_CASE(18)
+      SF_LANE_CASE(19) SF_LANE_CASE(20) SF_LANE_CASE(21) SF_LANE_CASE(22)
+      SF_LANE_CASE(23)
+      default:
+        set_error("sf_kl_fit: no masked lane kernel for this number of directions");
+        return SF_EINVAL;
+    }
+#undef SF_LANE_CASE
+    static_assert(kLaneMaskedMaxD == 23, "the cases above");
+    SF_HIP(hipGetLastError());
+  }
 #define SF_LANE_CASE(d)                                                        \
   case d:                                                                      \
     launch_lane<d>(ctx, p, r, S, A, phase, coef, resid, w_out, order_out);     \
diff --git a/ska-sdp-screen-fitting_amd/csrc/kl_fit_pool.h b/ska-sdp-screen-fitting_amd/csrc/kl_fit_pool.h
--- a/ska-sdp-screen-fitting_amd/csrc/kl_fit_pool.h
+++ b/ska-sdp-screen-fitting_amd/csrc/kl_fit_pool.h
@@ -394,7 +394,8 @@
 
 constexpr int kAncestorMinMasks = 8192;
 
-static int number_and_decompose(sf_ctx* ctx, int* n_slow, int* n_nonuniform) {
+static int number_and_decompose(sf_ctx* ctx, int* n_slow, int* n_nonuniform,
+                                int* n_ids = nullptr) {
   SF_HIP(hipMemcpyAsync(ctx->d_counters + kCntPassStart, ctx->d_counters + kCntIds,
                         sizeof(int), hipMemcpyDeviceToDevice, ctx->stream));
   SF_HIP(hipMemsetAsync(ctx->d_counters + kCntMaxLevel, 0, sizeof(int), ctx->stream));
@@ -410,6 +411,7 @@
   SF_HIP(hipStreamSynchronize(ctx->stream));
   *n_slow = cnt[kCntSlow];
   *n_nonuniform = cnt[kCntNonUniform];
+  if (n_ids) *n_ids = cnt[kCntIds];
   if (cnt[kCntIds] > old_cap) {
     SF_TRY(ensure_pool(ctx, (size_t)cnt[kCntIds]));
     hipLaunchKernelGGL(kl_fill_mask_kernel, dim3((cap + 255) / 256), dim3(256),
diff --git a/ska-sdp-screen-fitting_amd/csrc/sf_internal.h b/ska-sdp-screen-fitting_amd/csrc/sf_internal.h
--- a/ska-sdp-screen-fitting_amd/csrc/sf_internal.h
+++ b/ska-sdp-screen-fitting_amd/csrc/sf_internal.h
@@ -118,6 +118,8 @@
   kCntLaneDeferred = 7,
   kCntLane = 8,
   kCntList = 9,
+  kCntLaneMasked = 10,
+  kCntLaneMaskedDeferred = 11,
 };
 constexpr int kFitCounters = 12;
 enum FitError {
@@ -198,6 +200,8 @@
   sf::DevBuf<int> d_pos;
   sf::DevBuf<uint8_t> d_class;
   sf::DevBuf<long long> d_list;
+  sf::DevBuf<long long> d_glist;
+  sf::DevBuf<int> d_mask_bins;
   sf::DevBuf<double> d_sigma;
   sf::DevBuf<int> d_counters;
   sf::DevBuf<double> d_scratch;
@@ -223,6 +227,8 @@
   int fit_pack = 1;
   int fit_lean = 1;
   int fit_lane = 1;
+  int fit_lane_masked = 1;
+  int fit_lane_mask_min = 0;
 };
 
 namespace sf {
diff --git a/ska-sdp-screen-fitting_amd/ska_sdp_screen_fitting_amd/_lib.py b/ska-sdp-screen-fitting_amd/ska_sdp_screen_fitting_amd/_lib.py
--- a/ska-sdp-screen-fitting_amd/ska_sdp_screen_fitting_amd/_lib.py
+++ b/ska-sdp-screen-fitting_amd/ska_sdp_screen_fitting_amd/_lib.py
@@ -43,6 +43,8 @@
 SF_OPT_FIT_WIDE_POOL_MB = 20
 SF_OPT_FIT_WIDE_POOL_MAX = 21
 SF_OPT_FIT_LANE = 22
+SF_OPT_FIT_LANE_MASKED = 23
+SF_OPT_FIT_LANE_MASK_MIN = 24
 SF_EVAL_KERNEL_AUTO = 0
 SF_EVAL_KERNEL_TILE = 1
 SF_EVAL_KERNEL_LDS4 = 2
@@ -66,7 +68,7 @@
 EXPORTED = (
     "sf_version", "sf_last_error", "sf_create", "sf_destroy", "sf_set_stream",
     "sf_synchronize", "sf_set_option", "sf_get_eval_kernel", "sf_get_eval_contraction", "sf_alloc", "sf_free", "sf_copy_h2d", "sf_copy_d2h",
-    "sf_set_basis", "sf_set_basis_wide", "sf_set_piercepoints", "sf_get_basis", "sf_kl_fit", "sf_get_fit_stats", "sf_get_fit_lane_stats", "sf_get_fit_pool",
+    "sf_set_basis", "sf_set_basis_wide", "sf_set_piercepoints", "sf_get_basis", "sf_kl_fit", "sf_get_fit_stats", "sf_get_fit_lane_stats", "sf_get_fit_lane_masked_stats", "sf_get_fit_pool",
     "sf_get_fit_pool_wide",
     "sf_stream_create", "sf_stream_destroy", "sf_device_cus",
     "sf_set_grid", "sf_kl_eval", "sf_kl_eval_gain", "sf_kl_eval_sums",
@@ -145,6 +147,7 @@
                            ctypes.POINTER(FitParams), vp, vp, vp, vp], c_int),
             "sf_get_fit_stats": ([vp, ip, ip], c_int),
             "sf_get_fit_lane_stats": ([vp, ctypes.POINTER(i64), ctypes.POINTER(i64)], c_int),
+            "sf_get_fit_lane_masked_stats": ([vp, ctypes.POINTER(i64), ctypes.POINTER(i64)], c_int),
             "sf_get_fit_pool": ([vp, vp, vp, c_int, ip], c_int),
             "sf_get_fit_pool_wide": ([vp, vp, vp, c_int, ip], c_int),
             "sf_set_grid": ([vp, vp, c_int, vp, c_int], c_int),
@@ -339,6 +342,12 @@
                "sf_get_fit_lane_stats")
         return {"n_lane": nl.value, "n_deferred": nd.value}
 
+    def fit_lane_masked_stats(self):
+        nm, nd = ctypes.c_int64(), ctypes.c_int64()
+        _check(self.lib.sf_get_fit_lane_masked_stats(self.h, ctypes.byref(nm), ctypes.byref(nd)),
+               "sf_get_fit_lane_masked_stats")
+        return {"n_masked": nm.value, "n_deferred": nd.value}
+
     def fit_pool(self):
         n = ctypes.c_int(0)
         _check(self.lib.sf_get_fit_pool(self.h, None, None, 0, ctypes.byref(n)),
```

Measured after the change: 6.308 million (median of 6 runs). Within noise of the previous version (+0.3%).
